# KennyRotella/delta_graph_slam

Measured on AMD Instinct MI355X. Metric: scan registrations/sec (64k-pt pairs), higher is better.
Workload: dtype f32 per-point, f64 accumulate; 1 GPU; cfg2 KITTI HDL-64E-shaped pairs (65,536 pts after voxel filter), NDT res 1.0 m DIRECT7, eps 0.01, max 64 iterations; 32 candidate pairs per GPU per step against one target (LoopDetector::matching, cfg4 shard), 32 distinct source scans, fitness score per candidate; inputs resident on the device before timing -- the 35 MB working set of a step fits the 256 MB Infinity Cache, so re-reads between eval; pairs_per_gpu=32, distinct_scans=32, parallelism=candidates sharded one process per GPU, all_gather of result records, collective_world_size=1

## Files before the change

delta_graph_slam_amd/csrc/dgs_api.hip:

```cpp
#include <algorithm>
#include <cfloat>
#include <cmath>
#include <cstddef>
#include <cstdlib>
#include <cstring>
#include <new>

#include "handle.h"

using namespace dgs;

namespace dgs {

int ensure_pinned(dgs_handle* h, size_t bytes) {
  if (bytes <= h->pinned_bytes) return DGS_OK;
  if (h->pinned) (void)hipHostFree(h->pinned);
  h->pinned = nullptr;
  h->pinned_bytes = 0;
  const size_t want = std::max<size_t>(bytes * 2, 1 << 16);
  hipError_t e = hipHostMalloc(&h->pinned, want, hipHostMallocDefault);
  if (e != hipSuccess) {
    h->err = std::string("hipHostMalloc: ") + hipGetErrorString(e);
    return DGS_ERR_HIP;
  }
// ... 252 lines not shown
  p->ndt_min_points_per_voxel = 6;
  p->ndt_line_search = DGS_NDT_LS_MORE_THUENTE;
  p->ndt_mt_max_step_iterations = 10;
  p->ndt_fix_hessian_d1 = 0;
  p->ndt_strict_order = DGS_NDT_ORDER_UPSTREAM;
  p->ndt_newton_solver = 1;
  p->ndt_hessian_recompute_double = 1;
  p->ndt_guess_rotation_polar = 1;
  p->ndt_exp_glibc = 1;
  p->ndt_cov_eigensolver = 1;
  p->gicp_cov_jacobi_svd = 0;
  p->gicp_max_correspondence_distance = 2.5;
  p->gicp_rotation_epsilon = 2e-3;
  p->gicp_lm_init_lambda_factor = 1e-9;
  p->gicp_correspondence_randomness = 20;
  p->gicp_regularization = DGS_GICP_REG_PLANE;
  p->gicp_optimizer = DGS_GICP_OPT_LEVENBERG_MARQUARDT;
  p->gicp_lm_max_iterations = 10;
  p->vgicp_search_method = DGS_VGICP_DIRECT1;
  p->vgicp_resolution = 1.0;
  if (method == DGS_METHOD_PCL_NDT) p->ndt_search_method = DGS_NDT_KDTREE;
  return valid_method(method) ? DGS_OK : DGS_ERR_INVALID_ARGUMENT;
}

int dgs_pcl_gicp_options_init(dgs_pcl_gicp_options* o) {
  if (!o) return DGS_ERR_INVALID_ARGUMENT;
  std::memset(o, 0, sizeof(*o));
  o->struct_size = sizeof(dgs_pcl_gicp_options);
  o->max_optimizer_iterations = 20;
  o->rotation_epsilon = 2e-3;
  o->gicp_epsilon = 1e-3;
  o->use_reciprocal_correspondences = 0;
  return DGS_OK;
}

int dgs_set_pcl_gicp_options(dgs_handle* h, const dgs_pcl_gicp_options* o) {
  if (!h || !o || o->struct_size != sizeof(dgs_pcl_gicp_options)) return DGS_ERR_INVALID_ARGUMENT;
  h->err.clear();
  if (h->prm.method != DGS_METHOD_PCL_GICP) { h->err = "dgs_set_pcl_gicp_options: not a GICP_HIP handle"; return DGS_ERR_UNSUPPORTED; }
  if (o->max_optimizer_iterations < 1 || !(o->rotation_epsilon > 0) || !(o->gicp_epsilon >= 0)) {
    h->err = "dgs_set_pcl_gicp_options: max_optimizer_iterations >= 1, rotation_epsilon > 0 and gicp_epsilon >= 0 are required";
    return DGS_ERR_INVALID_ARGUMENT;
  }
  h->pg_opt = *o;
  return DGS_OK;
}

int dgs_pcl_gicp_set_correspondence_randomness(dgs_handle* h, int32_t k) {
  if (!h || k < 1) return DGS_ERR_INVALID_ARGUMENT;
  h->err.clear();
  if (h->prm.method != DGS_METHOD_PCL_GICP) { h->err = "dgs_pcl_gicp_set_correspondence_randomness: not a GICP_HIP handle"; return DGS_ERR_UNSUPPORTED; }
  h->prm.gicp_correspondence_randomness = k;
  return DGS_OK;
}

int dgs_pcl_gicp_get_trajectory(dgs_handle* h, int32_t pair, float* T16s, int32_t* n_corr, int32_t* inner, int32_t* passes, double* f, int32_t capacity,
                                int32_t* len) {
  if (!h || !len || pair < 0 || capacity < 0) return DGS_ERR_INVALID_ARGUMENT;
  h->err.clear();
  if (set_device(h)) return DGS_ERR_HIP;
  if (h->prm.method != DGS_METHOD_PCL_GICP) return DGS_ERR_UNSUPPORTED;
  int n = 0;
  int rc = pcl_gicp_trajectory(h, pair, T16s, n_corr, inner, passes, f, capacity, &n);
  *len = n;
  return rc;
}

int dgs_pcl_gicp_set_probe(dgs_handle* h, const float* T16, const float* guess16) {
  if (!h) return DGS_ERR_INVALID_ARGUMENT;
  h->err.clear();
  if (h->prm.method != DGS_METHOD_PCL_GICP) return DGS_ERR_UNSUPPORTED;
  std::memcpy(h->pg_probe_T, T16 ? T16 : kIdentity16, sizeof(h->pg_probe_T));
  std::memcpy(h->pg_probe_guess, guess16 ? guess16 : kIdentity16, sizeof(h->pg_probe_guess));
  return DGS_OK;
}

int dgs_pcl_gicp_evaluate(dgs_handle* h, const double* x6, int32_t* m, double* f, double* g6) {
  if (!h || !x6 || !m || !f || !g6) return DGS_ERR_INVALID_ARGUMENT;
  h->err.clear();
  if (set_device(h)) return DGS_ERR_HIP;
  if (h->prm.method != DGS_METHOD_PCL_GICP) return DGS_ERR_UNSUPPORTED;
  if (!h->have_target || h->nt == 0) return DGS_ERR_NO_TARGET;
  if (!h->have_source || h->ns == 0) return DGS_ERR_NO_SOURCE;
  return pcl_gicp_evaluate(h, x6, m, f, g6);
}

int dgs_icp_options_init(dgs_icp_options* o) {
  if (!o) return DGS_ERR_INVALID_ARGUMENT;
  std::memset(o, 0, sizeof(*o));
  o->struct_size = sizeof(dgs_icp_options);
  o->use_reciprocal_correspondences = 0;
  o->euclidean_fitness_epsilon = -DBL_MAX;
  o->rotation_epsilon = 0.0;
  return DGS_OK;
}

int dgs_set_icp_options(dgs_handle* h, const dgs_icp_options* o) {
  if (!h || !o || o->struct_size != sizeof(dgs_icp_options)) return DGS_ERR_INVALID_ARGUMENT;
  h->err.clear();
  if (h->prm.method != DGS_METHOD_ICP) { h->err = "dgs_set_icp_options: not an ICP handle"; return DGS_ERR_UNSUPPORTED; }
  h->icp_opt = *o;
  return DGS_OK;
}

int dgs_icp_get_trajectory(dgs_handle* h, int32_t pair, float* T16s, double* mse, int32_t* n_corr, int32_t capacity, int32_t* len) {
  if (!h || !len || pair < 0 || capacity < 0) return DGS_ERR_INVALID_ARGUMENT;
  h->err.clear();
  if (set_device(h)) return DGS_ERR_HIP;
  if (h->prm.method != DGS_METHOD_ICP) return DGS_ERR_UNSUPPORTED;
  int n = 0;
  int rc = icp_trajectory(h, pair, T16s, mse, n_corr, capacity, &n);
  *len = n;
  return rc;
}

int dgs_create(const dgs_params* params, dgs_handle** out) {
  if (!params || !out || params->struct_size != sizeof(dgs_params)) return DGS_ERR_INVALID_ARGUMENT;
  if (!valid_method(params->method)) return DGS_ERR_INVALID_ARGUMENT;
  if (params->method == DGS_METHOD_VGICP && (!(params->vgicp_resolution > 0) || params->vgicp_search_method < 0 || params->vgicp_search_method > DGS_VGICP_DIRECT27))
    return DGS_ERR_INVALID_ARGUMENT;
  if (!(params->ndt_resolution > 0) || params->maximum_iterations < 0 || params->gicp_correspondence_randomness < 1) return DGS_ERR_INVALID_ARGUMENT;
  if (params->ndt_strict_order < DGS_NDT_ORDER_FAST || params->ndt_strict_order > DGS_NDT_ORDER_UPSTREAM_SEQUENTIAL) return DGS_ERR_INVALID_ARGUMENT;
  *out = nullptr;
  dgs_handle* h = new (std::nothrow) dgs_handle();
  if (!h) return DGS_ERR_HIP;
  h->prm = *params;
  if (params->method == DGS_METHOD_PCL_NDT) {
    h->prm.ndt_search_method = DGS_NDT_KDTREE;
    h->prm.ndt_strict_order = DGS_NDT_ORDER_UPSTREAM;
    h->prm.ndt_hessian_recompute_double = 1;
  }
  int dev = params->device;
  hipError_t e = hipSuccess;
  if (dev < 0) e = hipGetDevice(&dev);
  if (e == hipSuccess) e = hipSetDevice(dev);
  if (e == hipSuccess) e = hipStreamCreateWithFlags(&h->stream, hipStreamNonBlocking);
  if (e != hipSuccess) {
    g_create_error = std::string("dgs_create(device=") + std::to_string(params->device) + "): " + hipGetErrorString(e);
    delete h;
    return DGS_ERR_HIP;
  }
  h->device = dev;
  h->own_stream = true;
  (void)side_create(h);
  if (kExperiments)
    if (const char* e = std::getenv("DGS_NN_GRID")) { h->grid_mode = std::atoi(e); h->grid_levels = std::max(1, std::atoi(e)); }
  if (const char* e = std::getenv("DGS_NDT_FUSED")) h->ndt_fused = std::atoi(e) != 0;
  if (const char* e = std::getenv("DGS_NDT_STRICT_KERNEL")) h->strict_kernel = std::atoi(e) == 2 ? 2 : 3;
  if (const char* e = std::getenv("DGS_NDT_HD_OVERLAP")) h->hd_overlap = std::atoi(e) != 0;
  if (const char* e = std::getenv("DGS_NDT_SOLVE_MIN_ACTIVE")) h->solve_min_active = std::max(0, std::atoi(e));
  if (const char* e = std::getenv("DGS_NDT_SPECULATE")) h->ndt_speculate = std::atoi(e) != 0;
  if (const char* e = std::getenv("DGS_NDT_FIXED_SLICES")) h->ndt_fixed_slices = std::atoi(e) != 0;
  if (const char* e = std::getenv("DGS_NDT_DEAL_BY_COST")) h->ndt_deal_by_cost = std::atoi(e) != 0;
  if (const char* e = std::getenv("DGS_NDT_QUEUE")) h->ndt_queue_mode = std::atoi(e);
  if (const char* e = std::getenv("DGS_NDT_SCHEDULE")) h->ndt_schedule = std::atoi(e) != 0;
  if (const char* e = std::getenv("DGS_NDT_QUEUE_MIN_PAIRS")) h->ndt_queue_min_pairs = std::max(1, std::atoi(e));
  if (const char* e = std::getenv("DGS_EARLY_FITNESS")) h->early_fitness_enabled = std::atoi(e) != 0;
  if (const char* e = std::getenv("DGS_EARLY_FITNESS_LDS_KB")) h->early_fit.lds_kb = std::max(0, std::atoi(e));
  if (const char* e = std::getenv("DGS_EARLY_FITNESS_MAX_ACTIVE")) h->early_fit.max_active = std::max(0, std::atoi(e));
  if (const char* e = std::getenv("DGS_EARLY_FITNESS_MIN_PAIRS")) h->early_fit.min_pairs = std::max(1, std::atoi(e));
  if (const char* e = std::getenv("DGS_NN_KD")) h->nn_kd = std::atoi(e) != 0;
  if (const char* e = std::getenv("DGS_NN_KD_ALL")) h->nn_kd_all = std::atoi(e) != 0;
  if (const char* e = std::getenv("DGS_NN_KD_MIN_QUERIES")) h->nn_kd_min_queries = std::atoll(e);
  if (const char* e = std::getenv("DGS_KNN_PARTS")) { const int v = std::atoi(e); h->knn_parts = (v == 1 || v == 2 || v == 4 || v == 8) ? v : 0; }
  if (const char* e = std::getenv("DGS_KNN_LEAF")) h->knn_leaf = std::atoi(e) != 0;
  if (const char* e = std::getenv("DGS_KNN_MIN_WAVES")) h->knn_min_waves = std::max(1, std::atoi(e));
  if (const char* e = std::getenv("DGS_KNN_ROUNDS")) h->knn_rounds = std::max(1, std::atoi(e));
  if (const char* e = std::getenv("DGS_GICP_FUSED")) h->gicp_fused = std::atoi(e) != 0;
  if (kExperiments)
    if (const char* e = std::getenv("DGS_NDT_PACK2")) h->ndt_pack2 = std::atoi(e) != 0;
  if (const char* e = std::getenv("DGS_NN_GRID_FACTOR")) h->grid_spacing_factor = std::max(0.5f, (float)std::atof(e));
  std::memset(h->final_T, 0, sizeof(h->final_T));
  h->final_T[0] = h->final_T[5] = h->final_T[10] = h->final_T[15] = 1.f;
  (void)dgs_icp_options_init(&h->icp_opt);
  (void)dgs_pcl_gicp_options_init(&h->pg_opt);
  *out = h;
  return DGS_OK;
}

void dgs_destroy(dgs_handle* h) {
  if (!h) return;
  (void)hipSetDevice(h->device);
  (void)hipStreamSynchronize(h->stream);
  unbind(h, h->tgt_cloud);
  unbind(h, h->src_cloud);
  h->own_target.release(); h->own_source.release();
  for (int k = 0; k < 2; k++)
    if (h->ev_poll[k]) (void)hipEventDestroy(h->ev_poll[k]);
  if (h->hd_stream) {
    (void)hipStreamSynchronize(h->hd_stream);
    (void)hipStreamDestroy(h->hd_stream);
    for (int k = 0; k < dgs_handle::kHdEvents; k++) {
      if (h->ev_hd_a[k]) (void)hipEventDestroy(h->ev_hd_a[k]);
      if (h->ev_hd_b[k]) (void)hipEventDestroy(h->ev_hd_b[k]);
    }
  }
  if (h->side_stream) {
    (void)hipStreamSynchronize(h->side_stream);
    (void)hipStreamDestroy(h->side_stream);
    (void)hipEventDestroy(h->ev_fork);
    (void)hipEventDestroy(h->ev_join);
  }
  h->batch_slab.release();
  for (auto& c : h->batch_clouds) c.release();
  icp_release(h);
  pcl_gicp_release(h);
  prefilter_release(h);
  map_cloud_release(h);
  line_extraction_release(h);
  line_align_release(h);
  line_align_local_release(h);
  line_edges_release(h);
  building_overlap_release(h);
  floor_detection_release(h);
  fitness_batch_release(h);
  building_cloud_release(h);
  h->gitems.release(); h->vvox.release(); h->vcell2vox.release();
  h->cell2vox.release(); h->vox.release(); h->vox_centroid.release(); h->vox_dbg.release(); h->vox_strict.release(); h->vox_count.release(); h->vox_valid.release();
  h->key_in.release(); h->key_out.release(); h->val_in.release(); h->val_out.release(); h->run_keys.release();
  h->run_counts.release(); h->run_offsets.release(); h->dev_scalars.release(); h->vg_run_keys.release(); h->vg_scalars.release(); h->minmax_partial.release(); h->cub_temp.release();
  h->pairs.release(); h->inits.release(); h->partials.release(); h->done_counter.release(); h->ndt_queue.release(); h->ndt_ring.release(); h->pair_blocks.release(); h->src_ptrs.release(); h->src_sizes.release();
  h->nn_partials.release(); h->scratch_cloud.release(); h->strict_rows.release(); h->strict_totals.release(); h->tgt_grid.release(); h->aux_grid.release();
  h->fc_in.release(); h->fc_out.release(); h->fc_cnt.release();
  h->aux_cloud1.release(); h->aux_cloud2.release(); h->aux_out.release(); h->aux_bvh.release();
  h->corr.release(); h->corr_sq.release(); h->mahal.release(); h->gpairs.release(); h->slice_blk_pair.release(); h->slice_rows.release();
  for (auto& ep : h->prof.pool) { (void)hipEventDestroy(ep.start); (void)hipEventDestroy(ep.stop); }
  if (h->pinned) (void)hipHostFree(h->pinned);
  if (h->done_flags) (void)hipHostFree(h->done_flags);
  if (h->fit_host) (void)hipHostFree(h->fit_host);
  if (h->own_stream && h->stream) (void)hipStreamDestroy(h->stream);
  delete h;
}

const char* dgs_last_error(const dgs_handle* h) { return h ? h->err.c_str() : g_create_error.c_str(); }

int dgs_set_stream(dgs_handle* h, void* hip_stream) {
  if (!h) return DGS_ERR_INVALID_ARGUMENT;
  h->err.clear();
  if (set_device(h)) return DGS_ERR_HIP;
  DGS_HIP_TRY(h, hipStreamSynchronize(h->stream));
  if (h->own_stream && h->stream) (void)hipStreamDestroy(h->stream);
  if (hip_stream) {
    h->stream = reinterpret_cast<hipStream_t>(hip_stream);
    h->own_stream = false;
  } else {
    DGS_HIP_TRY(h, hipStreamCreateWithFlags(&h->stream, hipStreamNonBlocking));
    h->own_stream = true;
  }
  return DGS_OK;
}

int dgs_synchronize(dgs_handle* h) {
  if (!h) return DGS_ERR_INVALID_ARGUMENT;
  h->err.clear();
  if (set_device(h)) return DGS_ERR_HIP;
  DGS_HIP_TRY(h, hipStreamSynchronize(h->stream));
  return DGS_OK;
}

int dgs_set_input_target(dgs_handle* h, const float* xyz16, int64_t n, int32_t on_device) {
  if (!h || n < 0 || (n > 0 && !xyz16) || n > INT32_MAX) return DGS_ERR_INVALID_ARGUMENT;
  h->err.clear();
  if (set_device(h)) return DGS_ERR_HIP;
  h->have_target = false;
  h->vmap_valid = false;
  h->tgt_grid.valid = false;
  unbind(h, h->tgt_cloud);
  h->tgt = &h->own_target;
  h->tgt->invalidate();
  h->tgt->n = n;
  h->nt = n;
  int rc = upload_cloud(h, h->own_target.pts, xyz16, n, on_device);
  if (rc) return rc;
  if (is_ndt_family(h)) {
    rc = ndt_build_target(h);
    if (rc) return rc;
  }
  h->have_target = true;
  return DGS_OK;
}

int dgs_set_input_source(dgs_handle* h, const float* xyz16, int64_t n, int32_t on_device) {
  if (!h || n < 0 || (n > 0 && !xyz16) || n > INT32_MAX) return DGS_ERR_INVALID_ARGUMENT;
  h->err.clear();
  if (set_device(h)) return DGS_ERR_HIP;
  h->have_source = false;
  unbind(h, h->src_cloud);
  h->src = &h->own_source;
  h->src->invalidate();
  h->src->n = n;
  h->ns = n;
  int rc = upload_cloud(h, h->own_source.pts, xyz16, n, on_device);
  if (rc) return rc;
  h->have_source = true;
  return DGS_OK;
}

int dgs_cloud_create(dgs_handle* h, const float* xyz16, int64_t n, int32_t on_device, dgs_cloud** out) {
  if (!h || !out || n < 0 || (n > 0 && !xyz16) || n > INT32_MAX) return DGS_ERR_INVALID_ARGUMENT;
  h->err.clear();
  *out = nullptr;
  if (set_device(h)) return DGS_ERR_HIP;
  dgs_cloud* c = new (std::nothrow) dgs_cloud();
  if (!c) return DGS_ERR_HIP;
  c->device = h->device;
  c->st.n = n;
  int rc = upload_cloud(h, c->st.pts, xyz16, n, on_device);
  if (rc != DGS_OK) {
    c->st.release();
    delete c;
    return rc;
  }
  *out = c;
  return DGS_OK;
}

void dgs_cloud_destroy(dgs_cloud* c) {
  if (!c) return;
  for (dgs_handle* h : c->users) {
    if (h->tgt_cloud == c) { h->tgt_cloud = nullptr; h->tgt = &h->own_target; h->nt = 0; h->have_target = false; h->tgt_grid.valid = false; }
    if (h->src_cloud == c) { h->src_cloud = nullptr; h->src = &h->own_source; h->ns = 0; h->have_source = false; }
  }
  (void)hipSetDevice(c->device);
  (void)hipDeviceSynchronize();
  c->st.release();
  delete c;
}

int64_t dgs_cloud_size(const dgs_cloud* c) { return c ? c->st.n : 0; }

int dgs_set_input_target_cloud(dgs_handle* h, dgs_cloud* c) {
  if (!h || !c || c->device != h->device) return DGS_ERR_INVALID_ARGUMENT;
  h->err.clear();
  if (set_device(h)) return DGS_ERR_HIP;
  h->have_target = false;
  h->vmap_valid = false;
  h->tgt_grid.valid = false;
  bind(h, h->tgt_cloud, c);
  h->tgt = &c->st;
  h->nt = c->st.n;
  if (is_ndt_family(h)) {
    int rc = ndt_build_target(h);
    if (rc) return rc;
  }
  h->have_target = true;
  return DGS_OK;
}

int dgs_set_input_source_cloud(dgs_handle* h, dgs_cloud* c) {
  if (!h || !c || c->device != h->device) return DGS_ERR_INVALID_ARGUMENT;
  h->err.clear();
  bind(h, h->src_cloud, c);
  h->src = &c->st;
  h->ns = c->st.n;
  h->have_source = true;
  return DGS_OK;
}

static void fail_result(dgs_result* r, const float* guess, int status) {
  std::memcpy(r->final_transformation, guess ? guess : kIdentity16, sizeof(float) * 16);
  r->converged = 0;
  r->iterations = 0;
  r->evaluations = 0;
  r->status = status;
  r->score = 0.0;
  r->fitness = NAN;
}

int dgs_align(dgs_handle* h, const float* guess16, dgs_result* out, float* aligned, int32_t aligned_on_device) {
  if (!h || !out) return DGS_ERR_INVALID_ARGUMENT;
  h->err.clear();
  fail_result(out, guess16, DGS_OK);
  if (set_device(h)) { out->status = DGS_ERR_HIP; return DGS_ERR_HIP; }
// ... 49 lines not shown
  if (!h->have_target || h->nt == 0) return DGS_ERR_NO_TARGET;
  if (!h->have_source || h->ns == 0) return DGS_ERR_NO_SOURCE;
  double sum = 0;
  int64_t cnt = 0, inl = 0;
  int rc = nn_fitness(h, h->src->pts.ptr, h->ns, h->final_T, DBL_MAX, max_sq_dist, &sum, &cnt, &inl);
  if (rc) return rc;
  *fraction = (double)inl / (double)h->ns;
  return DGS_OK;
}

int dgs_nearest_search_target(dgs_handle* h, const float* queries, int64_t m, int32_t on_device, int32_t* indices, float* sq_dists) {
  if (!h || m < 0 || (m > 0 && (!queries || !indices || !sq_dists))) return DGS_ERR_INVALID_ARGUMENT;
  h->err.clear();
  if (set_device(h)) return DGS_ERR_HIP;
  if (!h->have_target || h->nt == 0) return DGS_ERR_NO_TARGET;
  if (m == 0) return DGS_OK;
  const float4* dq = reinterpret_cast<const float4*>(queries);
  int32_t* didx = indices;
  float* dsq = sq_dists;
  DevBuf<float4> q;
  DevBuf<int32_t> bi;
  DevBuf<float> bd;
  int rc = DGS_OK;
  if (!on_device) {
    if (q.reserve(m) != hipSuccess || bi.reserve(m) != hipSuccess || bd.reserve(m) != hipSuccess) { h->err = "hipMalloc failed"; rc = DGS_ERR_HIP; }
    if (!rc && hipMemcpyAsync(q.ptr, queries, (size_t)m * sizeof(float4), hipMemcpyHostToDevice, h->stream) != hipSuccess) { h->err = "hipMemcpyAsync failed"; rc = DGS_ERR_HIP; }
    dq = q.ptr; didx = bi.ptr; dsq = bd.ptr;
  }
  if (!rc) rc = nn_search(h, dq, m, didx, dsq);
  if (!rc && !on_device) {
    if (hipMemcpyAsync(indices, didx, (size_t)m * sizeof(int32_t), hipMemcpyDeviceToHost, h->stream) != hipSuccess ||
        hipMemcpyAsync(sq_dists, dsq, (size_t)m * sizeof(float), hipMemcpyDeviceToHost, h->stream) != hipSuccess) { h->err = "hipMemcpyAsync failed"; rc = DGS_ERR_HIP; }
  }
  (void)hipStreamSynchronize(h->stream);
  q.release(); bi.release(); bd.release();
  return rc;
}

int dgs_nn_fitness_distances(dgs_handle* h, const float* queries, int64_t m, int32_t on_device, float* sq_dists) {
  if (!h || m < 0 || (m > 0 && (!queries || !sq_dists))) return DGS_ERR_INVALID_ARGUMENT;
  h->err.clear();
  if (set_device(h)) return DGS_ERR_HIP;
  if (!h->have_target || h->nt == 0) return DGS_ERR_NO_TARGET;
  if (h->grid_mode == 0) return DGS_ERR_UNSUPPORTED;
  if (m == 0) return DGS_OK;
  h->use_grid = true;
  if (side_join(h) != DGS_OK) return DGS_ERR_HIP;
  int rc = ensure_target_index(h);
  if (rc) return rc;
  const float4* dq = reinterpret_cast<const float4*>(queries);
  float* dsq = sq_dists;
  DevBuf<float4> q;
  DevBuf<float> bd;
  if (!on_device) {
    if (q.reserve(m) != hipSuccess || bd.reserve(m) != hipSuccess) { h->err = "hipMalloc failed"; rc = DGS_ERR_HIP; }
    if (!rc && hipMemcpyAsync(q.ptr, queries, (size_t)m * sizeof(float4), hipMemcpyHostToDevice, h->stream) != hipSuccess) { h->err = "hipMemcpyAsync failed"; rc = DGS_ERR_HIP; }
    dq = q.ptr; dsq = bd.ptr;
  }
  if (!rc) rc = nn_grid_search(h, h->tgt_grid, h->tgt->bvh, dq, m, dsq);
  if (!rc && !on_device && hipMemcpyAsync(sq_dists, dsq, (size_t)m * sizeof(float), hipMemcpyDeviceToHost, h->stream) != hipSuccess) { h->err = "hipMemcpyAsync failed"; rc = DGS_ERR_HIP; }
  (void)hipStreamSynchronize(h->stream);
  q.release(); bd.release();
  return rc;
}

static int gicp_batch(dgs_handle* h, int n, CloudState* const* cs, const float* guesses16, int compute_fitness, double fitness_max_range,
                      dgs_result* results) {
  struct KdScope { dgs_handle* h; ~KdScope() { h->batch_kd = false; } } kd_scope{h};
  static const int kd_min = std::getenv("DGS_GICP_KD_MIN_CANDIDATES") ? std::atoi(std::getenv("DGS_GICP_KD_MIN_CANDIDATES")) : 10;
  h->batch_kd = h->nn_kd && n >= kd_min;
  const MethodOps& ops = kMethodOps[h->prm.method];
  int rc = ops.align_batch(h, n, cs, guesses16, results);
  if (rc == DGS_OK && compute_fitness) {
    DGS_HIP_TRY(h, h->src_ptrs.reserve(n));
    DGS_HIP_TRY(h, h->src_sizes.reserve(n));
    std::vector<const float4*> ptrs(n);
    std::vector<int> sz(n);
    int max_n = 0;
    for (int i = 0; i < n; i++) { ptrs[i] = cs[i]->pts.ptr; sz[i] = (int)cs[i]->n; max_n = std::max(max_n, sz[i]); }
    DGS_HIP_TRY(h, hipMemcpyAsync(h->src_ptrs.ptr, ptrs.data(), sizeof(void*) * n, hipMemcpyHostToDevice, h->stream));
    DGS_HIP_TRY(h, hipMemcpyAsync(h->src_sizes.ptr, sz.data(), sizeof(int) * n, hipMemcpyHostToDevice, h->stream));
    DGS_HIP_TRY(h, hipStreamSynchronize(h->stream));
    std::vector<double> sums(n);
    std::vector<int64_t> cnts(n), inl(n);
    size_t stride = 0;
    const float* dT = ops.final_transforms(h, &stride);
    rc = nn_fitness_batch(h, n, h->src_ptrs.ptr, h->src_sizes.ptr, max_n, dT, stride, fitness_max_range, 0.0, sums.data(), cnts.data(), inl.data());
    if (rc == DGS_OK)
      for (int i = 0; i < n; i++) results[i].fitness = cnts[i] > 0 ? sums[i] / (double)cnts[i] : DBL_MAX;
  }
  if (rc == DGS_OK) {
    for (int i = 0; i < n; i++)
      if (cs[i]->n <= 0) fail_result(&results[i], guesses16 ? guesses16 + 16 * i : nullptr, DGS_ERR_NO_SOURCE);
  }
  return rc;
}

int dgs_align_batch(dgs_handle* h, int32_t n, const float* const* sources, const int64_t* sizes, int32_t on_device, const float* guesses16,
                    int32_t compute_fitness, double fitness_max_range, dgs_result* results) {
  if (!h || n < 0 || (n > 0 && (!sources || !sizes || !results))) return DGS_ERR_INVALID_ARGUMENT;
  h->err.clear();
  if (set_device(h)) return DGS_ERR_HIP;
  if (n == 0) return DGS_OK;
  for (int i = 0; i < n; i++) fail_result(&results[i], guesses16 ? guesses16 + 16 * i : nullptr, DGS_OK);
  if (!h->have_target || h->nt == 0) {
    for (int i = 0; i < n; i++) results[i].status = DGS_ERR_NO_TARGET;
    h->err = "no input target dataset was given";
    return DGS_ERR_NO_TARGET;
  }
  if (!is_ndt_family(h)) {
    if (h->batch_clouds.size() < (size_t)n) h->batch_clouds.resize(n);
    std::vector<CloudState*> cs(n);
    for (int i = 0; i < n; i++) {
      if (sizes[i] < 0 || sizes[i] > INT32_MAX) return DGS_ERR_INVALID_ARGUMENT;
      CloudState& c = h->batch_clouds[i];
      c.invalidate();
      c.n = sources[i] ? sizes[i] : 0;
      int rc = upload_cloud(h, c.pts, sources[i], c.n, on_device);
      if (rc) return rc;
      cs[i] = &c;
    }
    return gicp_batch(h, n, cs.data(), guesses16, compute_fitness, fitness_max_range, results);
  }
  std::vector<const float4*> ptrs(n);
  std::vector<int> sz(n);
  DevBuf<float4>& slab = h->batch_slab;
  int64_t total = 0;
  for (int i = 0; i < n; i++) {
    if (sizes[i] < 0 || sizes[i] > INT32_MAX || (sizes[i] > 0 && !sources[i])) return DGS_ERR_INVALID_ARGUMENT;
    sz[i] = (int)sizes[i];
    total += sizes[i];
  }
  if (!on_device) {
    DGS_HIP_TRY(h, slab.reserve((size_t)std::max<int64_t>(total, 1)));
    int64_t off = 0;
    for (int i = 0; i < n; i++) {
      ptrs[i] = slab.ptr + off;
      if (sz[i]) DGS_HIP_TRY(h, hipMemcpyAsync(slab.ptr + off, sources[i], (size_t)sz[i] * sizeof(float4), hipMemcpyHostToDevice, h->stream));
      off += sz[i];
    }
  } else {
    for (int i = 0; i < n; i++) ptrs[i] = reinterpret_cast<const float4*>(sources[i]);
  }
  h->use_grid = grid_wanted(h, total);
  struct KdScope { dgs_handle* h; ~KdScope() { h->batch_kd = false; } } kd_scope{h};
  h->batch_kd = h->nn_kd && compute_fitness && total >= h->nn_kd_min_queries;
  if (compute_fitness && (!h->tgt->bvh.valid || (h->use_grid && !h->tgt_grid.valid)) && !h->prof.enabled) {
    int rs = side_fork(h);
    if (rs != DGS_OK) return rs;
    h->side_build_deferred = true;
  }
  int max_n = 0;
  for (int i = 0; i < n; i++) max_n = std::max(max_n, sz[i]);
  h->early_fit.on = h->early_fitness_enabled && compute_fitness && !h->prof.enabled && !h->use_grid && n <= 65535;
  h->early_fit.enqueued = false;
  h->early_fit.max_range = fitness_max_range;
  h->early_fit.max_n = max_n;
  int rc = ndt_align_pairs(h, n, ptrs.data(), sz.data(), guesses16, results);
  h->early_fit.on = false;
  if (side_join(h) != DGS_OK && rc == DGS_OK) rc = DGS_ERR_HIP;
  if (rc == DGS_OK && compute_fitness && h->early_fit.enqueued) {
    std::vector<double> sums(n);
    std::vector<int64_t> cnts(n), inl(n);
    nn_fitness_read(h, n, sums.data(), cnts.data(), inl.data());
    for (int i = 0; i < n; i++) results[i].fitness = cnts[i] > 0 ? sums[i] / (double)cnts[i] : DBL_MAX;
  } else if (rc == DGS_OK && compute_fitness) {
    std::vector<double> sums(n);
    std::vector<int64_t> cnts(n), inl(n);
    const float* dT = reinterpret_cast<const float*>(reinterpret_cast<const char*>(h->pairs.ptr) + offsetof(NdtPair, final_T));
    rc = nn_fitness_batch(h, n, h->src_ptrs.ptr, h->src_sizes.ptr, max_n, dT, sizeof(NdtPair), fitness_max_range, 0.0, sums.data(), cnts.data(),
                          inl.data());
    if (rc == DGS_OK)
      for (int i = 0; i < n; i++) results[i].fitness = cnts[i] > 0 ? sums[i] / (double)cnts[i] : DBL_MAX;
  }
  if (rc == DGS_OK) {
    for (int i = 0; i < n; i++)
      if (sz[i] == 0)
        fail_result(&results[i], guesses16 ? guesses16 + 16 * i : nullptr, DGS_ERR_NO_SOURCE);
  }
  (void)hipStreamSynchronize(h->stream);
  return rc;
}

int dgs_align_batch_clouds(dgs_handle* h, int32_t n, dgs_cloud* const* sources, const float* guesses16, int32_t compute_fitness,
                           double fitness_max_range, dgs_result* results) {
  if (!h || n < 0 || (n > 0 && (!sources || !results))) return DGS_ERR_INVALID_ARGUMENT;
  h->err.clear();
  if (set_device(h)) return DGS_ERR_HIP;
  if (n == 0) return DGS_OK;
  for (int i = 0; i < n; i++)
    if (!sources[i] || sources[i]->device != h->device) return DGS_ERR_INVALID_ARGUMENT;
  if (is_ndt_family(h)) {
    std::vector<const float*> ptrs(n);
    std::vector<int64_t> sizes(n);
    for (int i = 0; i < n; i++) { ptrs[i] = reinterpret_cast<const float*>(sources[i]->st.pts.ptr); sizes[i] = sources[i]->st.n; }
    return dgs_align_batch(h, n, ptrs.data(), sizes.data(), 1, guesses16, compute_fitness, fitness_max_range, results);
  }
  for (int i = 0; i < n; i++) fail_result(&results[i], guesses16 ? guesses16 + 16 * i : nullptr, DGS_OK);
  if (!h->have_target || h->nt == 0) {
    for (int i = 0; i < n; i++) results[i].status = DGS_ERR_NO_TARGET;
    h->err = "no input target dataset was given";
    return DGS_ERR_NO_TARGET;
  }
  std::vector<CloudState*> cs(n);
  for (int i = 0; i < n; i++) cs[i] = &sources[i]->st;
  return gicp_batch(h, n, cs.data(), guesses16, compute_fitness, fitness_max_range, results);
}

int dgs_profile_enable(dgs_handle* h, int32_t enable) {
  if (!h) return DGS_ERR_INVALID_ARGUMENT;
  if (set_device(h)) return DGS_ERR_HIP;
  prof_collect(h);
  h->prof.enabled = enable != 0;
  return DGS_OK;
}

int dgs_profile_get(dgs_handle* h, int32_t kernel_id, double* total_ms, int64_t* launches) {
  if (!h || kernel_id < 0 || kernel_id >= DGS_K_COUNT) return DGS_ERR_INVALID_ARGUMENT;
  if (set_device(h)) return DGS_ERR_HIP;
  prof_collect(h);
  if (total_ms) *total_ms = h->prof.total_ms[kernel_id];
  if (launches) *launches = h->prof.launches[kernel_id];
  return DGS_OK;
}

int dgs_profile_reset(dgs_handle* h) {
  if (!h) return DGS_ERR_INVALID_ARGUMENT;
  if (set_device(h)) return DGS_ERR_HIP;
  prof_collect(h);
  for (int k = 0; k < DGS_K_COUNT; k++) { h->prof.total_ms[k] = 0; h->prof.launches[k] = 0; }
  return DGS_OK;
}

int dgs_get_counts(dgs_handle* h, int64_t out[8]) {
  if (!h || !out) return DGS_ERR_INVALID_ARGUMENT;
  h->err.clear();
  if (set_device(h)) return DGS_ERR_HIP;
  for (int k = 0; k < 8; k++) out[k] = 0;
  out[0] = h->nt;
  out[1] = h->ns;
  if (is_ndt_family(h) && h->have_target && h->grid_cells > 0) {
    if (h->counts_stale) {
      int sc[2] = {0, 0};
      DGS_HIP_TRY(h, hipMemcpyAsync(sc, h->dev_scalars.ptr, sizeof(sc), hipMemcpyDeviceToHost, h->stream));
      DGS_HIP_TRY(h, hipStreamSynchronize(h->stream));
      h->n_occupied = sc[0];
      h->n_valid = sc[1];
      h->counts_stale = false;
    }
    out[2] = h->n_valid;
    out[3] = h->n_occupied;
    out[4] = h->grid_cells;
  }
  out[5] = h->last_evaluations;
  return DGS_OK;
}

int dgs_ndt_derivatives(dgs_handle* h, const double* p6, const float* T16, double* score, double* grad6, double* hess36) {
  if (!h || !p6 || !score || !grad6 || (!hess36 && !is_pcl_ndt(h))) return DGS_ERR_INVALID_ARGUMENT;
  h->err.clear();
  if (set_device(h)) return DGS_ERR_HIP;
  if (!is_ndt_family(h)) return DGS_ERR_UNSUPPORTED;
  if (!h->have_target || h->nt == 0) return DGS_ERR_NO_TARGET;
  if (!h->have_source || h->ns == 0) return DGS_ERR_NO_SOURCE;
  if (!hess36) {
    double unused[36];
    return ndt_probe(h, p6, T16, score, grad6, unused, 0);
  }
  return ndt_probe(h, p6, T16, score, grad6, hess36);
}

int dgs_pcl_ndt_neighbours(dgs_handle* h, const float* queries_xyz16, int64_t m, int32_t on_device, int32_t* counts, int32_t* voxel_ids) {
  if (!h || m < 0 || m > INT32_MAX || (m > 0 && (!queries_xyz16 || !counts || !voxel_ids))) return DGS_ERR_INVALID_ARGUMENT;
  h->err.clear();
  if (set_device(h)) return DGS_ERR_HIP;
  if (!is_pcl_ndt(h)) { h->err = "dgs_pcl_ndt_neighbours: not a PCL_NDT_HIP handle"; return DGS_ERR_UNSUPPORTED; }
  if (!h->have_target || h->nt == 0) return DGS_ERR_NO_TARGET;
  return pcl_ndt_neighbours(h, queries_xyz16, m, on_device, counts, voxel_ids);
}

int dgs_ndt_hessian_double(dgs_handle* h, const double* p6, double* hess36) {
  if (!h || !p6 || !hess36) return DGS_ERR_INVALID_ARGUMENT;
  h->err.clear();
  if (set_device(h)) return DGS_ERR_HIP;
  if (!is_ndt_family(h) || h->prm.ndt_strict_order == DGS_NDT_ORDER_FAST || !h->prm.ndt_hessian_recompute_double) return DGS_ERR_UNSUPPORTED;
  if (!h->have_target || h->nt == 0) return DGS_ERR_NO_TARGET;
  if (!h->have_source || h->ns == 0) return DGS_ERR_NO_SOURCE;
  double score, g6[6];
  return ndt_probe(h, p6, nullptr, &score, g6, hess36, 2);
}

int dgs_ndt_score_gradient(dgs_handle* h, const double* p6, double* score, double* grad6) {
  if (!h || !p6 || !score || !grad6) return DGS_ERR_INVALID_ARGUMENT;
  h->err.clear();
  if (set_device(h)) return DGS_ERR_HIP;
  if (!is_ndt_family(h) || is_pcl_ndt(h) || h->prm.ndt_strict_order == DGS_NDT_ORDER_FAST) return DGS_ERR_UNSUPPORTED;
  if (!h->have_target || h->nt == 0) return DGS_ERR_NO_TARGET;
  if (!h->have_source || h->ns == 0) return DGS_ERR_NO_SOURCE;
  double unused[36];
  return ndt_probe(h, p6, nullptr, score, grad6, unused, 0);
}

int dgs_deal_probe(dgs_handle* h, const int32_t* active, int32_t n_pairs, int32_t cap_blocks, int32_t grid, int32_t* out) {
  if (!h || !active || !out || n_pairs < 1 || cap_blocks < 1 || grid < n_pairs || grid > (1 << 20)) return DGS_ERR_INVALID_ARGUMENT;
  h->err.clear();
  if (set_device(h)) return DGS_ERR_HIP;
  DevBuf<int> d_active;
  DevBuf<int4> d_out;
  const size_t n_out = (size_t)grid * (kBlock / kWave);
  hipError_t e = d_active.reserve((size_t)n_pairs);
  if (e == hipSuccess) e = d_out.reserve(n_out);
  if (e == hipSuccess) e = hipMemcpyAsync(d_active.ptr, active, sizeof(int) * (size_t)n_pairs, hipMemcpyHostToDevice, h->stream);
  if (e == hipSuccess) {
    hipLaunchKernelGGL(deal_probe_kernel, dim3(grid), dim3(kBlock), 0, h->stream, d_active.ptr, n_pairs, cap_blocks, d_out.ptr);
    e = hipGetLastError();
  }
  if (e == hipSuccess) e = hipMemcpyAsync(out, d_out.ptr, sizeof(int4) * n_out, hipMemcpyDeviceToHost, h->stream);
  if (e == hipSuccess) e = hipStreamSynchronize(h->stream);
  d_active.release();
  d_out.release();
  if (e != hipSuccess) {
    h->err = std::string("dgs_deal_probe: ") + hipGetErrorString(e);
    return DGS_ERR_HIP;
  }
  return DGS_OK;
}

int dgs_deal_probe_cost(dgs_handle* h, const int32_t* active, const int32_t* kinds, int32_t n_pairs, int32_t cap_blocks, int32_t grid, int32_t* out, int32_t* order3) {
  if (!h || !active || !kinds || !out || n_pairs < 1 || cap_blocks < 1 || grid < n_pairs || grid > (1 << 20)) return DGS_ERR_INVALID_ARGUMENT;
  for (int32_t i = 0; i < n_pairs; i++)
    if (kinds[i] < 0 || kinds[i] > 2) return DGS_ERR_INVALID_ARGUMENT;
  h->err.clear();
  if (set_device(h)) return DGS_ERR_HIP;
  if (order3) { order3[0] = kNdtCostKind0; order3[1] = kNdtCostKind1; order3[2] = kNdtCostKind2; }
  DevBuf<int> d_in;
  DevBuf<int4> d_out;
  const size_t n_out = (size_t)grid * (kBlock / kWave);
  hipError_t e = d_in.reserve(2 * (size_t)n_pairs);
  if (e == hipSuccess) e = d_out.reserve(n_out);
  if (e == hipSuccess) e = hipMemcpyAsync(d_in.ptr, active, sizeof(int) * (size_t)n_pairs, hipMemcpyHostToDevice, h->stream);
  if (e == hipSuccess) e = hipMemcpyAsync(d_in.ptr + n_pairs, kinds, sizeof(int) * (size_t)n_pairs, hipMemcpyHostToDevice, h->stream);
  if (e == hipSuccess) {
    hipLaunchKernelGGL(deal_probe_cost_kernel, dim3(grid), dim3(kBlock), 0, h->stream, d_in.ptr, d_in.ptr + n_pairs, n_pairs, cap_blocks, d_out.ptr);
    e = hipGetLastError();
  }
  if (e == hipSuccess) e = hipMemcpyAsync(out, d_out.ptr, sizeof(int4) * n_out, hipMemcpyDeviceToHost, h->stream);
  if (e == hipSuccess) e = hipStreamSynchronize(h->stream);
  d_in.release();
  d_out.release();
  if (e != hipSuccess) {
    h->err = std::string("dgs_deal_probe_cost: ") + hipGetErrorString(e);
    return DGS_ERR_HIP;
  }
  return DGS_OK;
}

int dgs_find_loop_candidates(dgs_handle* h, const double* accum_distance, const double* xy, int64_t n, int32_t on_device, double new_accum_distance,
                             const double* new_xy, double accum_distance_thresh, double distance_thresh, int32_t* indices, int64_t capacity, int64_t* n_out) {
  if (!h || !n_out || !new_xy || n < 0 || capacity < 0 || (n > 0 && (!accum_distance || !xy)) || (capacity > 0 && !indices) || n > INT32_MAX) return DGS_ERR_INVALID_ARGUMENT;
  h->err.clear();
  if (set_device(h)) return DGS_ERR_HIP;
  *n_out = 0;
  if (n == 0) return DGS_OK;
  dgs::DevBuf<double>& din = h->fc_in;
  dgs::DevBuf<int>& dout = h->fc_out;
  dgs::DevBuf<long long>& dcnt = h->fc_cnt;
  const double* d_acc = accum_distance;
  const double* d_xy = xy;
  int* d_idx = indices;
  const int64_t cap = on_device ? capacity : std::min<int64_t>(capacity, n);
  if (dcnt.reserve(1) != hipSuccess) { h->err = "hipMalloc failed"; return DGS_ERR_HIP; }
  if (ensure_pinned(h, 8192) != DGS_OK) return DGS_ERR_HIP;
  long long* count = reinterpret_cast<long long*>(reinterpret_cast<char*>(h->pinned) + 4096);
  *count = 0;
  if (!on_device) {
    if (din.reserve((size_t)3 * n) != hipSuccess || dout.reserve((size_t)std::max<int64_t>(cap, 1)) != hipSuccess) { h->err = "hipMalloc failed"; return DGS_ERR_HIP; }
    DGS_HIP_TRY(h, hipMemcpyAsync(din.ptr, accum_distance, sizeof(double) * n, hipMemcpyHostToDevice, h->stream));
    DGS_HIP_TRY(h, hipMemcpyAsync(din.ptr + n, xy, sizeof(double) * 2 * n, hipMemcpyHostToDevice, h->stream));
    d_acc = din.ptr; d_xy = din.ptr + n; d_idx = dout.ptr;
  }
  hipLaunchKernelGGL(find_candidates_kernel, dim3(1), dim3(1024), 0, h->stream, d_acc, d_xy, (long long)n, new_accum_distance, new_xy[0], new_xy[1],
                     accum_distance_thresh, distance_thresh, d_idx, (long long)cap, dcnt.ptr);
  DGS_HIP_TRY(h, hipMemcpyAsync(count, dcnt.ptr, sizeof(long long), hipMemcpyDeviceToHost, h->stream));
  if (!on_device && cap > 0) DGS_HIP_TRY(h, hipMemcpyAsync(indices, d_idx, sizeof(int32_t) * (size_t)cap, hipMemcpyDeviceToHost, h->stream));
  DGS_HIP_TRY(h, hipStreamSynchronize(h->stream));
  if (hipGetLastError() != hipSuccess) { h->err = "find_candidates_kernel failed"; return DGS_ERR_HIP; }
  *n_out = *count;
  if (*count > capacity) { h->err = "indices buffer too small for the candidates"; return DGS_ERR_INVALID_ARGUMENT; }
  return DGS_OK;
}

int dgs_calc_fitness_score(dgs_handle* h, const float* cloud1, int64_t n1, const float* cloud2, int64_t n2, int32_t on_device,
                           const float* relpose16, double max_range, double* score) {
  if (!h || !score || n1 < 0 || n2 < 0 || (n1 > 0 && !cloud1) || (n2 > 0 && !cloud2) || n1 > INT32_MAX || n2 > INT32_MAX) return DGS_ERR_INVALID_ARGUMENT;
  h->err.clear();
  if (set_device(h)) return DGS_ERR_HIP;
  *score = DBL_MAX;
  if (n1 == 0 || n2 == 0) return DGS_OK;
  int rc = upload_cloud(h, h->aux_cloud1, cloud1, n1, on_device);
  if (rc == DGS_OK) rc = upload_cloud(h, h->aux_cloud2, cloud2, n2, on_device);
  if (rc == DGS_OK) rc = bvh_build(h, h->aux_bvh, h->aux_cloud1.ptr, n1);
  const bool aux_grid = grid_wanted(h, n2);
  if (rc == DGS_OK && aux_grid) rc = nn_grid_build(h, h->aux_grid, h->aux_bvh, h->aux_cloud1.ptr, n1);
  if (rc != DGS_OK) return rc;
  hipStream_t st = h->stream;
// ... 172 lines not shown
```

delta_graph_slam_amd/csrc/handle.h:

```cpp
#pragma once
#include "building_cloud.h"
#include "common.h"
#include "sac.h"

namespace dgs {

struct EventPair {
  hipEvent_t start, stop;
};

struct Profiler {
  bool enabled = false;
  std::vector<EventPair> pool;
  std::vector<int> pending[DGS_K_COUNT];
  size_t next_free = 0;
  double total_ms[DGS_K_COUNT] = {0};
  int64_t launches[DGS_K_COUNT] = {0};
};

struct IcpPair;
struct IcpItem;
struct PgPair;
struct PgItem;
struct PgInit;
// ... 134 lines not shown
  DevBuf<LaHyp> hyps;
  DevBuf<unsigned char> keep, gate;
  DevBuf<int> blk, cnt, surv, slot;
  DevBuf<double> fit;
  DevBuf<LaResult> result;
  int64_t n_hyp = 0;
  int64_t counts4[4] = {0, 0, 0, 0};
};
struct LalHyp;
struct LalScratch {
  DevBuf<unsigned char> in;
  DevBuf<unsigned char> tab;
  DevBuf<LalHyp> hyps;
  DevBuf<double> fit;
  DevBuf<double> keys;
  DevBuf<double> base;
  DevBuf<unsigned char> out;
  std::vector<int64_t> off1, off2;
  int64_t counts8[8] = {0, 0, 0, 0, 0, 0, 0, 0};
};
struct LeSeg;
struct LeScratch {
  DevBuf<double> lines;
  DevBuf<LeSeg> segs;
  DevBuf<unsigned char> cnt;
  DevBuf<int> blk;
  DevBuf<int> eoff;
  DevBuf<double> edges;
  void* stage = nullptr;
  size_t stage_bytes = 0;
  std::vector<int> eoff_host;
  int64_t counts4[4] = {0, 0, 0, 0};
};
struct BoHyp;
struct BoScratch {
  DevBuf<unsigned char> in;
  DevBuf<double> shr;
  DevBuf<unsigned long long> bits;
  DevBuf<int> row;
  DevBuf<unsigned char> out;
  DevBuf<unsigned char> ain;
  DevBuf<BoHyp> hyps;
  DevBuf<unsigned char> aout;
  std::vector<int64_t> off;
  int64_t counts8[8] = {0, 0, 0, 0, 0, 0, 0, 0};
};

struct FdHyp;
struct FdScratch {
  DevBuf<float4> in, tilted, clipped, kept, filtered;
  DevBuf<unsigned char> flags, nflags;
  DevBuf<int> blk, cnt;
  CloudState cloud;
  DevBuf<int> nbr;
  DevBuf<float4> normals;
  DevBuf<float> cov9;
  SacScratch sac;
  DevBuf<FdHyp> hyps;
  std::vector<float4> host_filtered;
  std::vector<int32_t> inliers;
  int64_t n_clipped = 0, n_filtered = 0;
  bool have_normals = false;
  dgs_floor_detection_trace trace{};
};

struct FbEdge;
struct FbSeg;
struct FbScratch {
  DevBuf<unsigned char> tab;
  DevBuf<double> rows;
  void* stage = nullptr;
  size_t stage_bytes = 0;
  DevBuf<FbSeg> segs;
  DevBuf<float> mm;
  DevBuf<unsigned long long> keys, keys_alt;
  DevBuf<uint32_t> vals, vals_alt;
  void* bstage = nullptr;
  size_t bstage_bytes = 0;
  hipEvent_t ev_bstage = nullptr;
  bool bstage_pending = false;
  int64_t counts8[8] = {0, 0, 0, 0, 0, 0, 0, 0};
};

struct BcScratch {
  bc::StepTable steps;
  int64_t table_on_device = 0;
  DevBuf<float> table;
  DevBuf<unsigned char> in;
  DevBuf<float4> rec;
  DevBuf<int> cnt;
  DevBuf<int> item_off;
  DevBuf<float4> out;
  int64_t n_out = 0, n_items = -1;
  int64_t counts8[8] = {0, 0, 0, 0, 0, 0, 0, 0};
};

}

struct dgs_handle;
struct dgs_cloud {
  dgs::CloudState st;
  int device = 0;
  std::vector<dgs_handle*> users;
};

struct dgs_handle {
  dgs_params prm;
  int device = 0;
  hipStream_t stream = nullptr;
  bool own_stream = false;
  hipEvent_t ev_poll[2] = {nullptr, nullptr};
  hipStream_t side_stream = nullptr;
  hipEvent_t ev_fork = nullptr, ev_join = nullptr;
  hipStream_t hd_stream = nullptr;
  static constexpr int kHdEvents = 32;
  hipEvent_t ev_hd_a[kHdEvents] = {}, ev_hd_b[kHdEvents] = {};
  int strict_kernel = 3;
  bool hd_overlap = true;
  bool ndt_speculate = true;
  bool ndt_fixed_slices = false;
  bool ndt_deal_by_cost = true;
#ifdef DGS_DEAL_STAMPS
  unsigned long long* deal_stamps = nullptr;
  long long deal_stamp_seq = 0;
#endif
  int solve_min_active = 0;
  bool side_pending = false;
  bool side_build_deferred = false;
  std::string err;

  dgs::CloudState own_target, own_source;
  dgs::CloudState* tgt = &own_target;
  dgs::CloudState* src = &own_source;
  dgs_cloud* tgt_cloud = nullptr;
  dgs_cloud* src_cloud = nullptr;
  int64_t nt = 0, ns = 0;
  bool have_target = false, have_source = false;

  dgs::VoxelGrid grid{};
  dgs::DevBuf<int> cell2vox;
  dgs::DevBuf<dgs::VoxelRec> vox;
  dgs::DevBuf<float4> vox_centroid;
  dgs::DevBuf<double> vox_dbg;
  dgs::DevBuf<dgs::VoxelStrictRec> vox_strict;
  dgs::DevBuf<int> vox_count;
  dgs::DevBuf<int> vox_valid;
  dgs::DevBuf<uint32_t> key_in, key_out, val_in, val_out, run_keys;
  dgs::DevBuf<int> run_counts, run_offsets;
  dgs::DevBuf<int> dev_scalars;
  dgs::DevBuf<uint32_t> vg_run_keys;
  dgs::DevBuf<int> vg_scalars;
  dgs::DevBuf<float> minmax_partial;
  dgs::DevBuf<unsigned char> cub_temp;
  int64_t grid_cells = 0;
  int64_t n_occupied = 0, n_valid = 0;
  int64_t n_occupied_bound = 0;
  bool counts_stale = true;

  dgs::DevBuf<dgs::NdtPair> pairs;
  dgs::DevBuf<dgs::NdtInit> inits;
  dgs::DevBuf<double> partials;
  dgs::DevBuf<int> done_counter;
  int* done_flags = nullptr;
  int done_flags_cap = 0;
  dgs::DevBuf<int> ndt_queue;
  dgs::DevBuf<unsigned char> ndt_ring;
  int ndt_ring_rounds = 0;
  int ndt_queue_mode = 0;
  bool ndt_schedule = false;
  int ndt_queue_min_pairs = 2;
  dgs::DevBuf<int> pair_blocks;
  dgs::DevBuf<double> strict_rows;
  dgs::DevBuf<double> strict_totals;
  dgs::DevBuf<const float4*> src_ptrs;
  dgs::DevBuf<int> src_sizes;
  dgs::NdtConsts consts{};
  int64_t last_evaluations = 0;
  dgs::DevBuf<int> knn_nbr;
  dgs::DevBuf<int> knn_stats;
  bool nn_kd = true;
  int64_t nn_kd_min_queries = 6 * 65536;
  bool nn_kd_all = false;
  bool batch_kd = false;
  int knn_parts = 0;
  bool knn_leaf = true;
  int knn_min_waves = 4096;
  int knn_rounds = 8;
  bool gicp_fused = true;
  bool ndt_pack2 = false;
  bool ndt_fused = true;

  void* pinned = nullptr;
  size_t pinned_bytes = 0;

  float final_T[16];
  bool have_result = false;

  dgs::DevBuf<double> nn_partials;
  int nn_bpp = 0;
  double* fit_host = nullptr;
  int fit_host_cap = 0;
  struct EarlyFitness {
    bool on = false;
    bool enqueued = false;
    double max_range = 0.0;
    int max_n = 0;
    int lds_kb = 0;
    int max_active = 1 << 30;
    int min_pairs = 8;
  } early_fit;
  bool early_fitness_enabled = false;
  const double* nn_out = nullptr;
  dgs::DevBuf<float4> scratch_cloud;
  dgs::NnGrid tgt_grid, aux_grid;
  int grid_mode = 0;
  bool use_grid = false;
  int grid_levels = 1;
  float grid_spacing_factor = 6.f;

  dgs::DevBuf<float4> aux_cloud1, aux_cloud2, aux_out;
  dgs::DevBuf<double> fc_in;
  dgs::DevBuf<int> fc_out;
  dgs::DevBuf<long long> fc_cnt;
  dgs::Bvh aux_bvh;
  int64_t bvh_builds = 0;

  dgs::DevBuf<int> corr;
  dgs::DevBuf<float> corr_sq;
  dgs::DevBuf<double> mahal;
  dgs::DevBuf<dgs::GicpPair> gpairs;
  dgs::DevBuf<dgs::GicpItem> gitems;
  dgs::VgicpMap vmap{};
  dgs::DevBuf<dgs::VgicpVoxel> vvox;
  dgs::DevBuf<int> vcell2vox;
  bool vmap_valid = false;
  int64_t vmap_voxels = 0;
  dgs::DevBuf<float4> batch_slab;
  std::vector<dgs::CloudState> batch_clouds;
  dgs::GicpConsts gconsts{};

  dgs::DevBuf<int> slice_blk_pair;
  dgs::DevBuf<double> slice_rows;

  dgs_icp_options icp_opt{};
  dgs::DevBuf<dgs::IcpPair> ipairs;
  dgs::DevBuf<dgs::IcpItem> iitems;
  dgs::DevBuf<float4> icp_w;
  dgs::DevBuf<int> icp_origin;
  dgs::DevBuf<float> icp_traj_T;
  dgs::DevBuf<double> icp_traj_mse;
  dgs::DevBuf<int> icp_traj_n;
  std::vector<dgs::Bvh> icp_w_bvh;
  std::vector<int> icp_last_iters;
  int icp_traj_cap = 0;

  dgs_pcl_gicp_options pg_opt{};
  dgs::DevBuf<dgs::PgPair> pgpairs;
  dgs::DevBuf<dgs::PgItem> pgitems;
  dgs::DevBuf<dgs::PgInit> pginits;
  dgs::DevBuf<float4> pg_w;
  dgs::DevBuf<float4> pg_q;
  dgs::DevBuf<double> pg_m;
  dgs::DevBuf<float> pg_traj_T;
  dgs::DevBuf<int> pg_traj_i;
  dgs::DevBuf<double> pg_traj_f;
  std::vector<int> pg_last_iters;
  int pg_traj_cap = 0;
  float pg_probe_T[16] = {1, 0, 0, 0, 0, 1, 0, 0, 0, 0, 1, 0, 0, 0, 0, 1};
  float pg_probe_guess[16] = {1, 0, 0, 0, 0, 1, 0, 0, 0, 0, 1, 0, 0, 0, 0, 1};

  dgs::PfScratch pf;

  dgs::McScratch mc;

  dgs::LnScratch ln;
  dgs::LaScratch la;
  dgs::LalScratch lal;
  dgs::LeScratch le;
  dgs::BoScratch bo;

  dgs::FdScratch fd;

  dgs::FbScratch fb;

  dgs::BcScratch bcl;

  dgs::Profiler prof;
};

namespace dgs {

int prof_begin(dgs_handle* h, int kernel_id, hipStream_t st = nullptr);
void prof_end(dgs_handle* h, int kernel_id, int slot, hipStream_t st = nullptr);
int ensure_pinned(dgs_handle* h, size_t bytes);
int ensure_poll_events(dgs_handle* h);
int side_fork(dgs_handle* h);
int side_join(dgs_handle* h);
int side_build_now(dgs_handle* h);

int ndt_build_target(dgs_handle* h);
int voxel_grid_filter(dgs_handle* h, const float4* in, int64_t n, float leaf, float4* out, int64_t out_capacity, int64_t* n_out);
int approx_voxel_grid_filter(dgs_handle* h, const float4* in, int64_t n, float leaf, float4* out, int64_t out_capacity, int64_t* n_out);
int cloud_minmax(dgs_handle* h, const float4* pts, int64_t n, float out6[6]);
int cloud_minmax_device(dgs_handle* h, const float4* pts, int64_t n, float** d_out6, hipStream_t st = nullptr);
int ndt_align_pairs(dgs_handle* h, int n_pairs, const float4* const* d_src_ptrs_host, const int* sizes_host,
                    const float* guesses16, dgs_result* results);
int ndt_trajectory(dgs_handle* h, int pair, double* out, int* len);
int ndt_probe(dgs_handle* h, const double* p6, const float* T16, double* score, double* g6, double* H36, int kind = 1);
inline bool is_pcl_ndt(const dgs_handle* h) { return h->prm.method == DGS_METHOD_PCL_NDT; }
inline bool is_ndt_family(const dgs_handle* h) { return h->prm.method == DGS_METHOD_NDT || h->prm.method == DGS_METHOD_PCL_NDT; }
void pcl_ndt_launch(dgs_handle* h, int n_pairs, int cap_blocks, int total_blocks, int launch, hipStream_t st);
void pcl_ndt_init_tables(dgs_handle* h, int n_pairs, hipStream_t st);
int pcl_ndt_neighbours(dgs_handle* h, const float* queries_xyz16, int64_t m, int on_device, int32_t* counts, int32_t* voxel_ids);
int bvh_build(dgs_handle* h, Bvh& bvh, const float4* pts, int64_t n, hipStream_t st = nullptr, bool kd_order = false);
int nn_fitness(dgs_handle* h, const float4* src, int64_t n, const float* T16, double max_range, double inlier_sq,
               double* sum, int64_t* count, int64_t* inliers);
int nn_fitness_batch(dgs_handle* h, int n_pairs, const float4* const* d_src_ptrs, const int* d_sizes, int max_size, const float* d_T,
                     size_t T_stride_bytes, double max_range, double inlier_sq, double* sums, int64_t* counts, int64_t* inliers);
int nn_fitness_batch_on(dgs_handle* h, const Bvh& index, NnGrid* grid, int n_pairs, const float4* const* d_src_ptrs, const int* d_sizes, int max_size,
                        const float* d_T, size_t T_stride_bytes, double max_range, double inlier_sq, double* sums, int64_t* counts, int64_t* inliers);
int nn_fitness_prepare(dgs_handle* h, int n_pairs, int max_size, bool grid);
void nn_fitness_enqueue(dgs_handle* h, hipStream_t st, const Bvh& index, const int* ids, int count, const float4* const* d_src_ptrs, const int* d_sizes,
                        const float* d_T, size_t T_stride_bytes, double max_range, double inlier_sq, int background_lds_kb);
int nn_fitness_totals_enqueue(dgs_handle* h, int n_pairs);
void nn_fitness_read(const dgs_handle* h, int n_pairs, double* sums, int64_t* counts, int64_t* inliers);
int nn_search(dgs_handle* h, const float4* queries, int64_t m, int32_t* d_idx, float* d_sq);
int ensure_target_index(dgs_handle* h, hipStream_t st = nullptr);
inline bool grid_wanted(const dgs_handle* h, int64_t queries) { return h->grid_mode > 0 || (h->grid_mode < 0 && queries >= 262144); }
#ifdef DGS_EXPERIMENTS
constexpr bool kExperiments = true;
int nn_grid_build(dgs_handle* h, NnGrid& G, const Bvh& bvh, const float4* pts, int64_t n, hipStream_t st = nullptr);
int nn_grid_launch_fitness(dgs_handle* h, NnGrid& G, const Bvh& index, int n_pairs, const float4* const* d_src_ptrs, const int* d_sizes, int max_n, const float* d_T,
                           size_t T_stride_bytes, float max_range, float inlier_sq, double* partial, int bpp);
int nn_grid_search(dgs_handle* h, NnGrid& G, const Bvh& index, const float4* queries, int64_t m, float* d_sq);
#else
constexpr bool kExperiments = false;
inline int nn_grid_build(dgs_handle*, NnGrid&, const Bvh&, const float4*, int64_t, hipStream_t = nullptr) { return DGS_ERR_UNSUPPORTED; }
inline int nn_grid_launch_fitness(dgs_handle*, NnGrid&, const Bvh&, int, const float4* const*, const int*, int, const float*, size_t, float, float, double*, int) { return DGS_ERR_UNSUPPORTED; }
inline int nn_grid_search(dgs_handle*, NnGrid&, const Bvh&, const float4*, int64_t, float*) { return DGS_ERR_UNSUPPORTED; }
#endif
int vgicp_build_map(dgs_handle* h);
int vgicp_voxels(dgs_handle* h, int64_t capacity, int32_t* coord3, int32_t* counts, double* mean3, double* cov9, int64_t* n_voxels);
int gicp_ensure_target_covariance(dgs_handle* h);
int gicp_align(dgs_handle* h, const float* guess16, dgs_result* out);
int gicp_align_batch(dgs_handle* h, int n, CloudState* const* srcs, const float* guesses16, dgs_result* out);
const float* gicp_final_transforms(dgs_handle* h, size_t* stride_bytes);
int gicp_covariances(dgs_handle* h, int which, double* host_out6, int64_t n);
int gicp_probe(dgs_handle* h, const double* T16_rowmajor, int error_only, double* err, double* H36, double* b6);
int icp_align(dgs_handle* h, const float* guess16, dgs_result* out);
int icp_align_batch(dgs_handle* h, int n, CloudState* const* srcs, const float* guesses16, dgs_result* out);
const float* icp_final_transforms(dgs_handle* h, size_t* stride_bytes);
int icp_trajectory(dgs_handle* h, int pair, float* T16s, double* mse, int32_t* n_corr, int capacity, int* len);
void icp_release(dgs_handle* h);
int knn_lists(dgs_handle* h, CloudState& c, int k, DevBuf<int>* out = nullptr);
void prefilter_release(dgs_handle* h);
void map_cloud_release(dgs_handle* h);
// ... 25 lines not shown
```

delta_graph_slam_amd/csrc/ndt_align.hip:

```cpp
#include <cfloat>
#include <cmath>
#include <cstdlib>
#include <cstring>

#include "handle.h"
#include "ndt_plan.h"
#include "solve6.h"

namespace dgs {

#include "ndt_fast.h"

#pragma clang fp contract(off)

#include "ndt_exp_tables.h"
#include "ndt_optimiser.h"
#include "ndt_strict.h"
#include "ndt_sequential.h"

__host__ __device__ inline int ndt_queue_slices(int round, int base, int cap) {
  const int f = round < 12 ? 1 : (round < 24 ? 2 : 4);
  return min(base * f, cap);
}
constexpr int kQueueHdrWords = 82;
static_assert(offsetof(NdtPair, need_hessian) == 81 * 4, "header layout");
constexpr size_t kQueueSlotBytes = 384;
__host__ __device__ inline NdtPair* queue_slot(char* ring, int ring_rounds, int pair, int round) {
  return reinterpret_cast<NdtPair*>(ring + ((size_t)pair * ring_rounds + round) * kQueueSlotBytes);
}
__device__ __forceinline__ unsigned long long* queue_word(int* queue, int pair) { return reinterpret_cast<unsigned long long*>(queue) + 1 + pair; }
__device__ __forceinline__ unsigned long long* queue_ctl(int* queue) { return reinterpret_cast<unsigned long long*>(queue); }
constexpr int kQueueStatInts = 16;

__global__ void ndt_init_kernel(NdtPair* __restrict__ pairs, const NdtInit* __restrict__ inits, int n_pairs, const NdtConsts c, int probe,
                                int* __restrict__ done_counter, const float4* const* __restrict__ stage_ptrs, const int* __restrict__ stage_sizes,
                                const float4** __restrict__ src_ptrs, int* __restrict__ src_sizes, int* __restrict__ queue, const int queue_slices0,
                                char* __restrict__ ring, const int ring_rounds) {
  const int i = blockIdx.x * blockDim.x + threadIdx.x;
  if (i < 16) done_counter[i] = 0;
  if (queue && i == 0) *queue_ctl(queue) = (unsigned long long)n_pairs;
  if (queue && i < kQueueStatInts) queue[2 * (n_pairs + 2) + i] = 0;
  if (i >= n_pairs) return;
  if (queue) *queue_word(queue, i) = (unsigned long long)queue_slices0 << 32;
  src_ptrs[i] = stage_ptrs[i];
  src_sizes[i] = stage_sizes[i];
  NdtPair* st = pairs + i;
  const NdtInit& in = inits[i];
  NdtSolver s;
  s.phase = probe ? PH_PROBE : PH_INIT_EVAL;
  s.nr_iterations = 0;
  s.trial_n = 0;
  s.trial_next = 0;
  s.evaluations = 0;
  s.converged = 0;
  s.step_iterations = 0;
  s.interval_converged = 0;
  s.open_interval = 1;
  s.traj_len = 1;
  s.score = 0;
  s.phi_0 = s.d_phi_0 = s.a_t = s.a_l = s.f_l = s.g_l = s.a_u = s.f_u = s.g_u = s.step_init = 0;
  for (int k = 0; k < 6; k++) { s.p[k] = in.p0[k]; s.grad[k] = 0; s.dir[k] = 0; st->traj[0][k] = in.p0[k]; }
  for (int k = 0; k < 36; k++) s.hess[k] = 0;
  double x[6];
  for (int k = 0; k < 6; k++) x[k] = in.p0[k];
  write_evaluation<false>(st, st, s, c, x, probe == 2 ? 2 : (probe == 3 ? 0 : 1), false, true);
  const float* G = in.guess;
  st->T[0] = G[0]; st->T[1] = G[4]; st->T[2] = G[8];  st->T[3] = G[12];
  st->T[4] = G[1]; st->T[5] = G[5]; st->T[6] = G[9];  st->T[7] = G[13];
  st->T[8] = G[2]; st->T[9] = G[6]; st->T[10] = G[10]; st->T[11] = G[14];
  for (int k = 0; k < 16; k++) st->final_T[k] = G[k];
  st->s = s;
  st->active = 1;
  st->last_launch = 0x7FFFFFFF;
  st->ticket = 0;
  st->serve[0] = 0;
  st->serve[1] = -1;
  st->serve[2] = -1;
  st->serve[3] = st->need_hessian & 3;
  st->spec_pending = 0;
  st->spec_result = 0;
  if (queue) {
    const int* from = reinterpret_cast<const int*>(st);
    int* to = reinterpret_cast<int*>(queue_slot(ring, ring_rounds, i, 0));
    for (int k = 0; k < kQueueHdrWords; k++) to[k] = from[k];
  }
}

struct NdtOut {
  float T[16];
  int converged, iterations, evaluations, pad;
  double score;
};

__global__ void ndt_export_kernel(const NdtPair* __restrict__ pairs, int n_pairs, NdtOut* __restrict__ out) {
  const int i = blockIdx.x * blockDim.x + threadIdx.x;
  if (i >= n_pairs) return;
  const NdtPair& st = pairs[i];
  NdtOut o;
  for (int k = 0; k < 16; k++) o.T[k] = st.final_T[k];
  o.converged = (st.s.phase == PH_DONE) ? st.s.converged : 0;
  o.iterations = st.s.nr_iterations;
  o.evaluations = st.s.evaluations;
  o.pad = 0;
  o.score = st.s.score;
  out[i] = o;
}

static void euler_angles_012(const float* T, float res[3]) {
  auto m = [&](int r, int c) { return T[c * 4 + r]; };
  const float kPi = 3.14159265358979323846f;
  res[0] = std::atan2(m(1, 2), m(2, 2));
  const float c2 = std::sqrt(m(0, 0) * m(0, 0) + m(0, 1) * m(0, 1));
  if (res[0] > 0.0f) {
    res[0] -= kPi;
    res[1] = std::atan2(-m(0, 2), -c2);
  } else {
    res[1] = std::atan2(-m(0, 2), c2);
  }
  const float s1 = std::sin(res[0]), c1 = std::cos(res[0]);
  res[2] = std::atan2(s1 * m(2, 0) - c1 * m(1, 0), c1 * m(1, 1) - s1 * m(2, 1));
  res[0] = -res[0];
  res[1] = -res[1];
  res[2] = -res[2];
}

static void affine_rotation_f32(const float* T_colmajor16, float* R) {
  constexpr int N = 3;
  const float precision = 2.f * FLT_EPSILON, tiny = FLT_MIN;
  float W[9], U[9], V[9];
  float scale = 0.f;
  for (int r = 0; r < 3; r++)
    for (int c = 0; c < 3; c++) { W[r * 3 + c] = T_colmajor16[c * 4 + r]; scale = std::fabs(W[r * 3 + c]) > scale ? std::fabs(W[r * 3 + c]) : scale; }
  if (scale == 0.f) scale = 1.f;
  for (int i = 0; i < 9; i++) { W[i] = W[i] / scale; U[i] = V[i] = (i % 4 == 0) ? 1.f : 0.f; }
  float max_diag = 0.f;
  for (int i = 0; i < N; i++) { const float a = std::fabs(W[i * 4]); if (a > max_diag) max_diag = a; }
  bool finished = false;
  for (int sweep = 0; sweep < 64 && !finished; sweep++) {
    finished = true;
    for (int p = 1; p < N; p++)
      for (int q = 0; q < p; q++) {
        const float pm = precision * max_diag;
        const float threshold = tiny > pm ? tiny : pm;
        if (!(std::fabs(W[p * N + q]) > threshold || std::fabs(W[q * N + p]) > threshold)) continue;
        finished = false;
        float m00 = W[p * N + p], m01 = W[p * N + q], m10 = W[q * N + p], m11 = W[q * N + q];
        const float t = m00 + m11, d = m10 - m01;
        float r1c, r1s;
        if (std::fabs(d) < tiny) { r1s = 0.f; r1c = 1.f; }
        else {
          const float u = t / d;
          const float tmp = std::sqrt(1.f + u * u);
          r1s = 1.f / tmp;
          r1c = u / tmp;
        }
        if (!(r1c == 1.f && r1s == 0.f)) {
          const float x0 = m00, y0 = m10, x1 = m01, y1 = m11;
          m00 = r1c * x0 + r1s * y0; m10 = -r1s * x0 + r1c * y0;
          m01 = r1c * x1 + r1s * y1; m11 = -r1s * x1 + r1c * y1;
        }
        float jrc, jrs;
        {
          const float deno = 2.f * std::fabs(m01);
          if (deno < tiny) { jrc = 1.f; jrs = 0.f; }
          else {
            const float tau = (m00 - m11) / deno;
            const float w = std::sqrt(tau * tau + 1.f);
            const float tt = (tau > 0.f) ? 1.f / (tau + w) : 1.f / (tau - w);
            const float sign_t = tt > 0.f ? 1.f : -1.f;
            const float nn = 1.f / std::sqrt(tt * tt + 1.f);
            jrs = -sign_t * (m01 / std::fabs(m01)) * std::fabs(tt) * nn;
            jrc = nn;
          }
        }
        const float jtc = jrc, jts = -jrs;
        const float jlc = r1c * jtc - r1s * jts;
        const float jls = r1c * jts + r1s * jtc;
        if (!(jlc == 1.f && jls == 0.f)) {
          for (int i = 0; i < N; i++) {
            const float xi = W[p * N + i], yi = W[q * N + i];
            W[p * N + i] = jlc * xi + jls * yi;
            W[q * N + i] = -jls * xi + jlc * yi;
          }
          for (int i = 0; i < N; i++) {
            const float xi = U[i * N + p], yi = U[i * N + q];
            U[i * N + p] = jlc * xi + jls * yi;
            U[i * N + q] = -jls * xi + jlc * yi;
          }
        }
        if (!(jrc == 1.f && -jrs == 0.f)) {
          const float c = jrc, s = -jrs;
// ... 125 lines not shown

#ifdef DGS_DEAL_STAMPS
static int deal_stamp_slot(dgs_handle* h, hipStream_t st) {
  static const char* file = std::getenv("DGS_DEAL_STAMPS_FILE");
  static const long long at = std::getenv("DGS_DEAL_STAMPS_AT") ? std::atoll(std::getenv("DGS_DEAL_STAMPS_AT")) : 2200;
  if (!file) return 0;
  const size_t words = (size_t)kStampLaunches * kStampGrid * kStampWords;
  const long long seq = h->deal_stamp_seq++;
  if (seq == at) {
    if (hipMalloc(reinterpret_cast<void**>(&h->deal_stamps), words * 8) != hipSuccess) { h->deal_stamps = nullptr; return 0; }
    (void)hipMemsetAsync(h->deal_stamps, 0, words * 8, st);
    (void)hipMemcpyToSymbolAsync(HIP_SYMBOL(g_deal_stamps), &h->deal_stamps, sizeof(h->deal_stamps), 0, hipMemcpyHostToDevice, st);
    (void)hipStreamSynchronize(st);
  }
  if (!h->deal_stamps || seq < at) return 0;
  if (seq < at + kStampLaunches) return (int)(seq - at) + 1;
  if (seq == at + kStampLaunches) {
    (void)hipStreamSynchronize(st);
    std::vector<unsigned long long> host(words);
    if (hipMemcpy(host.data(), h->deal_stamps, words * 8, hipMemcpyDeviceToHost) == hipSuccess) {
      if (FILE* f = std::fopen(file, "wb")) {
        std::fwrite(host.data(), 8, words, f);
        std::fclose(f);
      }
    }
  }
  return 0;
}
#endif

template <int SEARCH, bool FUSED, bool FIXED>
static void launch_strict_items(dgs_handle* h, const NdtPlan& P, const NdtLaunch& L, const dim3 grid, const int leaf_pow2, const int launch, hipStream_t st) {
  const int spec = (FUSED && P.speculate) ? 1 : 0;
  const dim3 grid_s(grid.x + (spec ? L.n_pairs : 0));
  int flags = (spec ? kStrictSpeculate : 0) | (h->ndt_deal_by_cost ? kStrictDealByCost : 0);
#ifdef DGS_DEAL_STAMPS
  flags |= deal_stamp_slot(h, st) << kStrictStampShift;
#endif
  hipLaunchKernelGGL((ndt_strict3_kernel<SEARCH, FUSED, true, FIXED>), grid_s, dim3(kBlock), 0, st, h->src_ptrs.ptr, h->src_sizes.ptr, h->pairs.ptr, h->grid, h->vox_strict.ptr,
                     h->vox_dbg.ptr, h->consts.gauss_d1, h->consts.gauss_d2, leaf_pow2, h->partials.ptr, L.n_pairs, L.cap_blocks, h->pair_blocks.ptr, h->consts,
                     FUSED ? h->done_flags : h->done_counter.ptr, launch, (FUSED && P.solve_beside) ? h->solve_min_active : 0, flags);
}

template <int SEARCH, bool FUSED, bool HD>
static void launch_strict_lanes(dgs_handle* h, const NdtPlan& P, const NdtLaunch& L, const dim3 grid, const int leaf_pow2, const int launch, hipStream_t st) {
  const int hd_lag = (FUSED && P.hd_overlap) ? 2 : 1;
  hipLaunchKernelGGL((ndt_strict_kernel<SEARCH, FUSED, HD>), grid, dim3(kBlock), 0, st, h->src_ptrs.ptr, h->src_sizes.ptr, h->pairs.ptr, h->grid, h->vox_strict.ptr,
                     h->vox_dbg.ptr, h->consts.gauss_d1, h->consts.gauss_d2, leaf_pow2, h->partials.ptr, L.n_pairs, L.cap_blocks, h->pair_blocks.ptr, h->consts,
                     FUSED ? h->done_flags : h->done_counter.ptr, launch, hd_lag);
}

template <int SEARCH, bool FUSED, bool PACK>
static void launch_fast(dgs_handle* h, const NdtLaunch& L, const dim3 grid, const int leaf_pow2, const int launch, hipStream_t st) {
  hipLaunchKernelGGL((ndt_derivatives_kernel<SEARCH, FUSED, PACK>), grid, dim3(kBlock), 0, st, h->src_ptrs.ptr, h->src_sizes.ptr, h->pairs.ptr, h->grid, h->consts.gauss_d1,
                     (float)h->consts.gauss_d2, leaf_pow2, h->partials.ptr, L.n_pairs, L.cap_blocks, h->pair_blocks.ptr, h->consts,
                     FUSED ? h->done_flags : h->done_counter.ptr, launch);
}

static void launch_derivatives(dgs_handle* h, const NdtPlan& P, const NdtLaunch& L, int launch = -1, bool hd = false) {
  const dim3 grid(L.total_blocks);
  int fe = 0;
  const int leaf_pow2 = (std::frexp(h->grid.leaf, &fe) == 0.5f) ? 1 : 0;
  const hipStream_t st = launch_stream(h, P, launch, hd);
  int slot = prof_begin(h, DGS_K_NDT_DERIVATIVES, st);
  if (is_pcl_ndt(h)) {
    if (!(hd && launch >= 0)) pcl_ndt_launch(h, L.n_pairs, L.cap_blocks, L.total_blocks, launch, st);
    prof_end(h, DGS_K_NDT_DERIVATIVES, slot, st);
    return;
  }
  with_search(P.search, [&](auto S) {
    constexpr int SEARCH = decltype(S)::value;
    if (P.order == DGS_NDT_ORDER_UPSTREAM_SEQUENTIAL) {
      launch_strict_rows<SEARCH>(h, L, grid, leaf_pow2, st);
    } else if (P.order == DGS_NDT_ORDER_UPSTREAM && P.item_kernel) {
      if (hd && launch >= 0) return;
      with_bool(launch >= 0, [&](auto FUSED) {
        with_bool(P.fixed_slices, [&](auto FIXED) { launch_strict_items<SEARCH, decltype(FUSED)::value, decltype(FIXED)::value>(h, P, L, grid, leaf_pow2, launch, st); });
      });
    } else if (P.order == DGS_NDT_ORDER_UPSTREAM) {
      with_bool(launch >= 0, [&](auto FUSED) {
        with_bool(hd, [&](auto HD) { launch_strict_lanes<SEARCH, decltype(FUSED)::value, decltype(HD)::value>(h, P, L, grid, leaf_pow2, launch, st); });
      });
    } else {
      with_bool(launch >= 0, [&](auto FUSED) {
        if constexpr (kExperiments && SEARCH == DGS_NDT_DIRECT7) {
          if (h->ndt_pack2) {
            launch_fast<SEARCH, decltype(FUSED)::value, true>(h, L, grid, leaf_pow2, launch, st);
            return;
          }
        }
        launch_fast<SEARCH, decltype(FUSED)::value, false>(h, L, grid, leaf_pow2, launch, st);
      });
    }
  });
  prof_end(h, DGS_K_NDT_DERIVATIVES, slot, st);
}

static void launch_solve(dgs_handle* h, const NdtPlan& P, const NdtLaunch& L) {
  int slot = prof_begin(h, DGS_K_NDT_SOLVE);
  hipLaunchKernelGGL(ndt_solve_kernel, dim3(L.n_pairs), dim3(kBlock), 0, h->stream, h->pairs.ptr, h->partials.ptr, L.cap_blocks, h->pair_blocks.ptr, h->consts,
                     h->done_counter.ptr, P.order != DGS_NDT_ORDER_FAST ? h->strict_totals.ptr : nullptr, P.order == DGS_NDT_ORDER_UPSTREAM ? 1 : 0);
  prof_end(h, DGS_K_NDT_SOLVE, slot);
}

static NdtLaunch choose_launch(int n_pairs, int max_n) {
  NdtLaunch L;
  L.n_pairs = n_pairs;
  static const int env_cap = std::getenv("DGS_NDT_CAP") ? std::atoi(std::getenv("DGS_NDT_CAP")) : 1024;
  static const int env_total = std::getenv("DGS_NDT_BLOCKS") ? std::atoi(std::getenv("DGS_NDT_BLOCKS")) : 1024;
  static const int env_ppt = std::getenv("DGS_NDT_PPT") ? std::max(1, std::atoi(std::getenv("DGS_NDT_PPT"))) : 2;
  static const int env_min = std::getenv("DGS_NDT_MIN_BLOCKS") ? std::max(1, std::atoi(std::getenv("DGS_NDT_MIN_BLOCKS"))) : 64;
  const int by_points = (max_n + kBlock * env_ppt - 1) / (kBlock * env_ppt);
  const int at_least = std::min(env_min, (max_n + kBlock - 1) / kBlock);
  L.cap_blocks = std::max(1, std::min({std::max(by_points, at_least), env_cap, kMaxPartialBlocks}));
  L.total_blocks = (int)std::max<int64_t>(n_pairs, std::min<int64_t>((int64_t)n_pairs * L.cap_blocks, env_total));
  L.max_n = std::max(max_n, 1);
  L.queue_workers = 0;
  L.queue_base = 0;
  return L;
}

static void choose_queue(dgs_handle* h, NdtLaunch& L) {
  static const int env_workers = std::getenv("DGS_NDT_QUEUE_WORKERS") ? std::atoi(std::getenv("DGS_NDT_QUEUE_WORKERS")) : 768;
  static const int env_base = std::getenv("DGS_NDT_QUEUE_BASE") ? std::atoi(std::getenv("DGS_NDT_QUEUE_BASE")) : 0;
  const int64_t most = (int64_t)L.n_pairs * L.cap_blocks;
  L.queue_workers = (int)std::max<int64_t>(1, std::min<int64_t>(env_workers, most));
  L.queue_base = env_base > 0 ? std::min(env_base, L.cap_blocks) : std::max(1, std::min(L.cap_blocks, L.queue_workers / std::max(1, L.n_pairs)));
  (void)h;
}

static int ndt_setup(dgs_handle* h, int n_pairs, const float4* const* src_ptrs_host, const int* sizes_host, const float* guesses16,
                     const double* probe_p6, NdtLaunch* launch_out, bool use_queue = false, int probe_kind = 1) {
  hipStream_t st = h->stream;
  fill_consts(h);
  int max_n = 0;
  for (int i = 0; i < n_pairs; i++) max_n = std::max(max_n, sizes_host[i]);
  NdtLaunch L = choose_launch(n_pairs, max_n);
  if (use_queue) {
    choose_queue(h, L);
    DGS_HIP_TRY(h, h->ndt_queue.reserve(2 * ((size_t)n_pairs + 2) + kQueueStatInts));
    const int per_iter_q = (h->prm.ndt_line_search == DGS_NDT_LS_FIXED_STEP && h->prm.ndt_step_size - h->prm.transformation_epsilon / 2 > 0) ? 1 : (h->prm.ndt_mt_max_step_iterations + 2);
    h->ndt_ring_rounds = (h->prm.maximum_iterations + 3) * per_iter_q + 8;
    DGS_HIP_TRY(h, h->ndt_ring.reserve((size_t)n_pairs * h->ndt_ring_rounds * kQueueSlotBytes));
  }
  *launch_out = L;
  DGS_HIP_TRY(h, h->pairs.reserve(n_pairs));
  DGS_HIP_TRY(h, h->inits.reserve(n_pairs));
  DGS_HIP_TRY(h, h->src_ptrs.reserve(n_pairs));
  DGS_HIP_TRY(h, h->src_sizes.reserve(n_pairs));
  DGS_HIP_TRY(h, h->partials.reserve((size_t)n_pairs * L.cap_blocks * (h->consts.strict_order ? kStrictPad : kAccumPad)));
  if (h->consts.strict_order) DGS_HIP_TRY(h, h->strict_totals.reserve((size_t)n_pairs * kStrictPad));
  if (h->consts.strict_order == DGS_NDT_ORDER_UPSTREAM_SEQUENTIAL) DGS_HIP_TRY(h, h->strict_rows.reserve((size_t)n_pairs * strict_rows_pair_stride(h, L)));
  DGS_HIP_TRY(h, h->pair_blocks.reserve(n_pairs));
  if (h->consts.strict_order == DGS_NDT_ORDER_UPSTREAM) DGS_HIP_TRY(h, hipMemsetAsync(h->pair_blocks.ptr, 0, sizeof(int) * n_pairs, st));
  DGS_HIP_TRY(h, h->done_counter.reserve(16));
  const size_t off_init = 256;
  const size_t off_ptr = off_init + sizeof(NdtInit) * n_pairs;
  const size_t off_size = off_ptr + sizeof(void*) * n_pairs;
  const size_t off_out = (off_size + sizeof(int) * n_pairs + 255) & ~(size_t)255;
  const size_t total = off_out + sizeof(NdtOut) * n_pairs + sizeof(NdtPair) + 256;
  if (ensure_pinned(h, total) != DGS_OK) return DGS_ERR_HIP;
  char* base = reinterpret_cast<char*>(h->pinned);
  NdtInit* hin = reinterpret_cast<NdtInit*>(base + off_init);
  const float ident[16] = {1, 0, 0, 0, 0, 1, 0, 0, 0, 0, 1, 0, 0, 0, 0, 1};
  for (int i = 0; i < n_pairs; i++) {
    const float* G = guesses16 ? guesses16 + 16 * i : ident;
    std::memcpy(hin[i].guess, G, sizeof(float) * 16);
    if (probe_p6) {
      for (int k = 0; k < 6; k++) hin[i].p0[k] = probe_p6[k];
    } else {
      float e[3];
      if (h->prm.ndt_guess_rotation_polar) {
        float R[9], Gp[16];
        affine_rotation_f32(G, R);
        std::memcpy(Gp, G, sizeof(Gp));
        for (int r = 0; r < 3; r++)
          for (int c = 0; c < 3; c++) Gp[c * 4 + r] = R[r * 3 + c];
        euler_angles_012(Gp, e);
      } else {
        euler_angles_012(G, e);
      }
      hin[i].p0[0] = G[12]; hin[i].p0[1] = G[13]; hin[i].p0[2] = G[14];
      hin[i].p0[3] = e[0]; hin[i].p0[4] = e[1]; hin[i].p0[5] = e[2];
    }
  }
  std::memcpy(base + off_ptr, src_ptrs_host, sizeof(void*) * n_pairs);
  std::memcpy(base + off_size, sizes_host, sizeof(int) * n_pairs);
  const size_t stage_bytes = off_size + sizeof(int) * n_pairs - off_init;
  DGS_HIP_TRY(h, h->inits.reserve((stage_bytes + sizeof(NdtInit) - 1) / sizeof(NdtInit)));
  DGS_HIP_TRY(h, hipMemcpyAsync(h->inits.ptr, hin, stage_bytes, hipMemcpyHostToDevice, st));
  const char* dstage = reinterpret_cast<const char*>(h->inits.ptr);
  hipLaunchKernelGGL(ndt_init_kernel, dim3((n_pairs + 63) / 64), dim3(64), 0, st, h->pairs.ptr, h->inits.ptr, n_pairs, h->consts, probe_p6 ? probe_kind : 0,
                     h->done_counter.ptr, reinterpret_cast<const float4* const*>(dstage + (off_ptr - off_init)),
                     reinterpret_cast<const int*>(dstage + (off_size - off_init)), h->src_ptrs.ptr, h->src_sizes.ptr,
                     L.queue_workers > 0 ? h->ndt_queue.ptr : nullptr, L.queue_workers > 0 ? ndt_queue_slices(0, L.queue_base, L.cap_blocks) : 0,
                     reinterpret_cast<char*>(h->ndt_ring.ptr), h->ndt_ring_rounds);
  if (is_pcl_ndt(h)) pcl_ndt_init_tables(h, n_pairs, st);
  return DGS_OK;
}

#ifdef DGS_EXPERIMENTS
#include "ndt_queue.h"
#else
static void launch_queue(dgs_handle*, const NdtLaunch&) {}
#endif

static int ndt_export(dgs_handle* h, int n_pairs, dgs_result* results);

int ndt_align_pairs(dgs_handle* h, int n_pairs, const float4* const* src_ptrs_host, const int* sizes_host, const float* guesses16,
                    dgs_result* results) {
  hipStream_t st = h->stream;
  NdtLaunch L{};
  const bool use_queue = kExperiments && h->ndt_queue_mode != 0 && h->ndt_fused && (h->consts.strict_order == DGS_NDT_ORDER_FAST) && n_pairs >= h->ndt_queue_min_pairs;
  int rc = ndt_setup(h, n_pairs, src_ptrs_host, sizes_host, guesses16, nullptr, &L, use_queue);
  if (rc != DGS_OK) return rc;
  const NdtPlan P = plan_align(h);
  if (use_queue) {
    launch_queue(h, L);
    if ((rc = side_build_now(h)) != DGS_OK) return rc;
    int* hq = reinterpret_cast<int*>(h->pinned);
    DGS_HIP_TRY(h, hipMemcpyAsync(hq, h->ndt_queue.ptr, sizeof(int) * 2, hipMemcpyDeviceToHost, st));
    rc = ndt_export(h, n_pairs, results);
    if (rc != DGS_OK) return rc;
#ifdef DGS_QUEUE_STATS
    {
      int q[8];
      (void)hipMemcpy(q, h->ndt_queue.ptr + 2 * (n_pairs + 2), sizeof(q), hipMemcpyDeviceToHost);
      int q2[8];
      (void)hipMemcpy(q2, h->ndt_queue.ptr + 2 * (n_pairs + 2) + 8, sizeof(q2), hipMemcpyDeviceToHost);
      const double it = std::max(1, q[4]);
      std::fprintf(stderr, "[queue] workers %d base %d: polls %d failed_claims %d claims %d closings %d; per worker: looking for work %.1f us, in items %.1f us; per item: %.2f us = record %.2f + "
                   "points %.2f + row %.2f + ticket %.2f; per closing %.2f us\n",
                   L.queue_workers, L.queue_base, q[2], q[3], q[4], q[7], q[5] * 0.01 / L.queue_workers, q[6] * 0.01 / L.queue_workers, q[6] * 0.01 / it, q2[0] * 0.01 / it,
                   q2[1] * 0.01 / it, q2[2] * 0.01 / it, q2[3] * 0.01 / it, q2[4] * 0.01 / std::max(1, q[7]));
    }
#endif
    if (hq[1] != 0 || hq[0] != 0) {
      h->err = "ndt_queue_kernel gave up (poll guard): " + std::to_string(hq[0]) + " registrations unfinished";
      return DGS_ERR_HIP;
    }
    return DGS_OK;
  }

  if (h->early_fit.on && (rc = nn_fitness_prepare(h, n_pairs, h->early_fit.max_n, false)) != DGS_OK) return rc;
  volatile int* flags = reinterpret_cast<volatile int*>(h->pinned);
  flags[0] = flags[1] = 0;
  if (ensure_poll_events(h) != DGS_OK) return DGS_ERR_HIP;
  const bool fused_flags = P.fused;
  if (fused_flags) {
    if (h->done_flags_cap < n_pairs) {
      if (h->done_flags) (void)hipHostFree(h->done_flags);
      h->done_flags = nullptr;
      h->done_flags_cap = 0;
      DGS_HIP_TRY(h, hipHostMalloc(reinterpret_cast<void**>(&h->done_flags), sizeof(int) * (size_t)(n_pairs + 64), hipHostMallocDefault));
      h->done_flags_cap = n_pairs + 64;
    }
    for (int i = 0; i < n_pairs; i++) h->done_flags[i] = 0;
  }
  hipEvent_t* ev = h->ev_poll;
  const bool fixed_one = h->prm.ndt_line_search == DGS_NDT_LS_FIXED_STEP && h->prm.ndt_step_size - h->prm.transformation_epsilon / 2 > 0;
  const int per_iter = fixed_one ? 1 : (h->prm.ndt_mt_max_step_iterations + 2);
  const long max_evals = ((long)(h->prm.maximum_iterations + 3) * per_iter + 2) * P.evals_factor;
  const int chunk = 4;
  long queued = 0;
  int launch_no = 0;
  const bool schedule = h->ndt_schedule;
  NdtLaunch Lq = L;
  if (schedule) choose_queue(h, Lq);
  int round_no = 0;
  int launches_upto[2] = {0, 0};
  int hd_rounds = 0;
  auto chained_round = [&](const NdtLaunch& Lr, auto&& beside) -> int {
    constexpr int R = dgs_handle::kHdEvents;
    if (launch_no >= 2) DGS_HIP_TRY(h, hipStreamWaitEvent(st, h->ev_hd_b[(launch_no - 2) % R], 0));
    launch_derivatives(h, P, Lr, launch_no);
    DGS_HIP_TRY(h, hipEventRecord(h->ev_hd_a[launch_no % R], st));
    DGS_HIP_TRY(h, hipStreamWaitEvent(h->hd_stream, h->ev_hd_a[launch_no % R], 0));
    beside();
    DGS_HIP_TRY(h, hipEventRecord(h->ev_hd_b[launch_no % R], h->hd_stream));
    hd_rounds = launch_no + 1;
    return DGS_OK;
  };
  auto enqueue_chunk = [&](int slot, int launches) -> int {
    for (int e = 0; e < launches; e++) {
      NdtLaunch Lr = L;
      if (schedule) {
        Lr.cap_blocks = ndt_queue_slices(round_no, Lq.queue_base, L.cap_blocks);
        Lr.total_blocks = n_pairs * Lr.cap_blocks;
      }
      round_no++;
      if (P.fused) {
        int rc_round = DGS_OK;
        if (P.two_kinds && P.hd_overlap) {
          rc_round = chained_round(Lr, [&] { launch_derivatives(h, P, Lr, launch_no, true); });
        } else if (P.solve_beside) {
          rc_round = chained_round(Lr, [&] {
            hipLaunchKernelGGL(ndt_strict_solve_kernel, dim3(n_pairs), dim3(kWave), 0, h->hd_stream, h->pairs.ptr, n_pairs, h->consts, h->done_flags, launch_no, 2);
          });
        } else {
          launch_derivatives(h, P, Lr, launch_no);
          if (P.two_kinds) launch_derivatives(h, P, Lr, launch_no, true);
        }
        if (rc_round != DGS_OK) return rc_round;
        launch_no++;
      } else {
        launch_derivatives(h, P, Lr);
        launch_solve(h, P, Lr);
        if (P.two_kinds) {
          launch_derivatives(h, P, Lr, -1, true);
          launch_solve(h, P, Lr);
        }
      }
    }
    queued += launches;
    launches_upto[slot] = launch_no;
    if (!fused_flags) DGS_HIP_TRY(h, hipMemcpyAsync(const_cast<int*>(&flags[slot]), h->done_counter.ptr, sizeof(int), hipMemcpyDeviceToHost, st));
    DGS_HIP_TRY(h, hipEventRecord(ev[slot], st));
    return DGS_OK;
  };
  auto pairs_done = [&](int slot) -> int {
    if (!fused_flags) return flags[slot];
    int n = 0;
    for (int i = 0; i < n_pairs; i++) n += reinterpret_cast<volatile int*>(h->done_flags)[i] != 0;
    return n;
  };
  const bool early = h->early_fit.on && fused_flags;
  std::vector<char> walked(early ? n_pairs : 0, 0);
  const float* fit_T = reinterpret_cast<const float*>(reinterpret_cast<const char*>(h->pairs.ptr) + offsetof(NdtPair, final_T));
  std::vector<int> ready;
  auto walk_finished = [&](int completed, bool rest) -> int {
    ready.clear();
    for (int i = 0; i < n_pairs; i++) {
      if (walked[i]) continue;
      const int f = reinterpret_cast<volatile int*>(h->done_flags)[i];
      if (rest || (f != 0 && f <= completed)) ready.push_back(i);
    }
    if (ready.empty() || (!rest && ((int)ready.size() < h->early_fit.min_pairs || n_pairs - pairs_done(0) > h->early_fit.max_active))) return DGS_OK;
    for (int i : ready) walked[i] = 1;
    nn_fitness_enqueue(h, rest ? st : h->side_stream, h->tgt->bvh, ready.data(), (int)ready.size(), h->src_ptrs.ptr, h->src_sizes.ptr, fit_T, sizeof(NdtPair),
                       h->early_fit.max_range, 0.0, rest ? 0 : h->early_fit.lds_kb);
    if (!rest) {
      DGS_HIP_TRY(h, hipEventRecord(h->ev_join, h->side_stream));
      h->side_pending = true;
    }
    return DGS_OK;
  };
  int cur = 0;
  rc = enqueue_chunk(0, h->side_build_deferred ? 2 * chunk : chunk);
  bool finished = false;
  bool first = true;
  while (rc == DGS_OK) {
    const bool more = queued < max_evals;
    if (more) rc = enqueue_chunk(cur ^ 1, chunk);
    if (rc != DGS_OK) break;
    if (first && (rc = side_build_now(h)) != DGS_OK) break;
    first = false;
    hipError_t e = hipEventSynchronize(ev[cur]);
    if (e != hipSuccess) { h->err = std::string("hipEventSynchronize: ") + hipGetErrorString(e); rc = DGS_ERR_HIP; break; }
    if (early && (rc = walk_finished(launches_upto[cur], false)) != DGS_OK) break;
    if (pairs_done(cur) >= n_pairs) { finished = true; break; }
    if (!more) break;
    cur ^= 1;
  }
  if (hd_rounds > 0) {
    hipError_t e = hipStreamWaitEvent(st, h->ev_hd_b[(hd_rounds - 1) % dgs_handle::kHdEvents], 0);
    if (e != hipSuccess && rc == DGS_OK) { h->err = std::string("hipStreamWaitEvent: ") + hipGetErrorString(e); rc = DGS_ERR_HIP; }
  }
  if (rc != DGS_OK) return rc;
  (void)finished;
  if (early) {
    if (side_join(h) != DGS_OK) return DGS_ERR_HIP;
    if ((rc = walk_finished(0, true)) != DGS_OK) return rc;
    if ((rc = nn_fitness_totals_enqueue(h, n_pairs)) != DGS_OK) return rc;
    h->early_fit.enqueued = true;
  }
  return ndt_export(h, n_pairs, results);
}

static int ndt_export(dgs_handle* h, int n_pairs, dgs_result* results) {
  hipStream_t st = h->stream;
  char* base = reinterpret_cast<char*>(h->pinned);
  const size_t off_out = ((256 + sizeof(NdtInit) * n_pairs + sizeof(void*) * n_pairs + sizeof(int) * n_pairs) + 255) & ~(size_t)255;
  NdtOut* hout = reinterpret_cast<NdtOut*>(base + off_out);
  NdtOut* dout = reinterpret_cast<NdtOut*>(h->partials.ptr);
  hipLaunchKernelGGL(ndt_export_kernel, dim3((n_pairs + 63) / 64), dim3(64), 0, st, h->pairs.ptr, n_pairs, dout);
  DGS_HIP_TRY(h, hipMemcpyAsync(hout, dout, sizeof(NdtOut) * n_pairs, hipMemcpyDeviceToHost, st));
  DGS_HIP_TRY(h, hipStreamSynchronize(st));
  DGS_HIP_TRY(h, hipGetLastError());
  int64_t evals = 0;
  for (int i = 0; i < n_pairs; i++) {
    std::memcpy(results[i].final_transformation, hout[i].T, sizeof(float) * 16);
    results[i].converged = hout[i].converged;
    results[i].iterations = hout[i].iterations;
    results[i].evaluations = hout[i].evaluations;
    results[i].status = DGS_OK;
    results[i].score = hout[i].score;
    results[i].fitness = NAN;
    evals += hout[i].evaluations;
  }
  h->last_evaluations = evals;
  return DGS_OK;
}

int ndt_trajectory(dgs_handle* h, int pair, double* out, int* len) {
  std::vector<char> buf(sizeof(NdtPair));
  DGS_HIP_TRY(h, hipStreamSynchronize(h->stream));
  DGS_HIP_TRY(h, hipMemcpy(buf.data(), h->pairs.ptr + pair, sizeof(NdtPair), hipMemcpyDeviceToHost));
  const NdtPair* st = reinterpret_cast<const NdtPair*>(buf.data());
#ifdef DGS_CLOSE_STAMPS
  const int n = kTrajCap;
#else
  const int n = std::min(st->s.traj_len, kTrajCap);
#endif
  for (int i = 0; i < n; i++)
    for (int k = 0; k < 6; k++) out[i * 6 + k] = st->traj[i][k];
  *len = n;
  return DGS_OK;
}

int ndt_probe(dgs_handle* h, const double* p6, const float* T16, double* score, double* g6, double* H36, int kind) {
  hipStream_t st = h->stream;
  NdtLaunch L{};
  const float4* src = h->src->pts.ptr;
  const int n = (int)h->ns;
  float T[16];
  if (T16) {
    std::memcpy(T, T16, sizeof(T));
  } else {
    const float rx = (float)p6[3], ry = (float)p6[4], rz = (float)p6[5];
    const float cx = (float)std::cos((double)rx), sx = (float)std::sin((double)rx), cy = (float)std::cos((double)ry), sy = (float)std::sin((double)ry),
                cz = (float)std::cos((double)rz), sz = (float)std::sin((double)rz);
    auto mul = [](float a, float b) { volatile float r = a * b; return (float)r; };
    T[0] = mul(cy, cz); T[4] = mul(-cy, sz); T[8] = sy; T[12] = (float)p6[0];
    { volatile float a = mul(cx, sz), b = mul(mul(sx, sy), cz); T[1] = a + b; }
    { volatile float a = mul(cx, cz), b = mul(mul(sx, sy), sz); T[5] = a - b; }
    T[9] = mul(-sx, cy); T[13] = (float)p6[1];
    { volatile float a = mul(sx, sz), b = mul(mul(cx, sy), cz); T[2] = a - b; }
    { volatile float a = mul(sx, cz), b = mul(mul(cx, sy), sz); T[6] = a + b; }
    T[10] = mul(cx, cy); T[14] = (float)p6[2];
    T[3] = T[7] = T[11] = 0.f; T[15] = 1.f;
  }
  int rc = ndt_setup(h, 1, &src, &n, T, p6, &L, false, kind == 0 ? 3 : kind);
  if (rc != DGS_OK) return rc;
  const NdtPlan P = plan_align(h);
  launch_derivatives(h, P, L, -1, kind == 2);
  launch_solve(h, P, L);
  char* base = reinterpret_cast<char*>(h->pinned);
  NdtPair* hp = reinterpret_cast<NdtPair*>(base + ((h->pinned_bytes - sizeof(NdtPair) - 64) & ~(size_t)63));
  DGS_HIP_TRY(h, hipMemcpyAsync(hp, h->pairs.ptr, sizeof(NdtPair), hipMemcpyDeviceToHost, st));
  DGS_HIP_TRY(h, hipStreamSynchronize(st));
  DGS_HIP_TRY(h, hipGetLastError());
  *score = hp->s.score;
  for (int k = 0; k < 6; k++) g6[k] = hp->s.grad[k];
  for (int k = 0; k < 36; k++) H36[k] = hp->s.hess[k];
  return DGS_OK;
}

}
```

delta_graph_slam_amd/csrc/ndt_voxel.hip:

```cpp
#include <hipcub/hipcub.hpp>

#include <cfloat>
#include <cmath>

#include "handle.h"
#include "small_linalg.h"

namespace dgs {

__global__ __launch_bounds__(kBlock) void minmax_kernel(const float4* __restrict__ pts, int64_t n, float* __restrict__ partial) {
  float mn[3] = {FLT_MAX, FLT_MAX, FLT_MAX}, mx[3] = {-FLT_MAX, -FLT_MAX, -FLT_MAX};
  for (int64_t i = blockIdx.x * (int64_t)blockDim.x + threadIdx.x; i < n; i += (int64_t)gridDim.x * blockDim.x) {
    const float4 p = pts[i];
    if (isfinite(p.x) && isfinite(p.y) && isfinite(p.z)) {
      mn[0] = fminf(mn[0], p.x); mn[1] = fminf(mn[1], p.y); mn[2] = fminf(mn[2], p.z);
      mx[0] = fmaxf(mx[0], p.x); mx[1] = fmaxf(mx[1], p.y); mx[2] = fmaxf(mx[2], p.z);
    }
  }
  __shared__ float sm[kBlock / kWave][6];
#pragma unroll
  for (int a = 0; a < 3; a++) {
#pragma unroll
    for (int off = 32; off > 0; off >>= 1) {
      mn[a] = fminf(mn[a], __shfl_down(mn[a], off, 64));
      mx[a] = fmaxf(mx[a], __shfl_down(mx[a], off, 64));
    }
  }
  const int lane = threadIdx.x & 63, wave = threadIdx.x >> 6;
  if (lane == 0)
    for (int a = 0; a < 3; a++) { sm[wave][a] = mn[a]; sm[wave][3 + a] = mx[a]; }
  __syncthreads();
  if (threadIdx.x < 6) {
    float v = sm[0][threadIdx.x];
    for (int w = 1; w < kBlock / kWave; w++) v = (threadIdx.x < 3) ? fminf(v, sm[w][threadIdx.x]) : fmaxf(v, sm[w][threadIdx.x]);
    partial[blockIdx.x * 6 + threadIdx.x] = v;
  }
}

__global__ void minmax_final_kernel(const float* __restrict__ partial, int nblocks, float* __restrict__ out6) {
  const int lane = threadIdx.x;
  float v[6] = {FLT_MAX, FLT_MAX, FLT_MAX, -FLT_MAX, -FLT_MAX, -FLT_MAX};
  for (int b = lane; b < nblocks; b += 64)
    for (int a = 0; a < 6; a++) v[a] = (a < 3) ? fminf(v[a], partial[b * 6 + a]) : fmaxf(v[a], partial[b * 6 + a]);
#pragma unroll
  for (int a = 0; a < 6; a++) {
#pragma unroll
    for (int off = 32; off > 0; off >>= 1) {
      const float o = __shfl_down(v[a], off, 64);
      v[a] = (a < 3) ? fminf(v[a], o) : fmaxf(v[a], o);
    }
  }
  if (lane == 0)
    for (int a = 0; a < 6; a++) out6[a] = v[a];
}

int cloud_minmax_device(dgs_handle* h, const float4* pts, int64_t n, float** d_out6, hipStream_t stream) {
  hipStream_t st = stream ? stream : h->stream;
  const int mm_blocks = (int)std::min<int64_t>((n + kBlock - 1) / kBlock, 256);
  DGS_HIP_TRY(h, h->minmax_partial.reserve((size_t)512 * 6 + 8));
  float* d_final = h->minmax_partial.ptr + (size_t)512 * 6;
  hipLaunchKernelGGL(minmax_kernel, dim3(mm_blocks), dim3(kBlock), 0, st, pts, n, h->minmax_partial.ptr);
  hipLaunchKernelGGL(minmax_final_kernel, dim3(1), dim3(64), 0, st, h->minmax_partial.ptr, mm_blocks, d_final);
  *d_out6 = d_final;
  return DGS_OK;
}

int cloud_minmax(dgs_handle* h, const float4* pts, int64_t n, float out6[6]) {
  hipStream_t st = h->stream;
  float* d_final = nullptr;
  int rc = cloud_minmax_device(h, pts, n, &d_final);
  if (rc) return rc;
  if (ensure_pinned(h, 4096) != DGS_OK) return DGS_ERR_HIP;
  float* hmm = reinterpret_cast<float*>(h->pinned);
  DGS_HIP_TRY(h, hipMemcpyAsync(hmm, d_final, 6 * sizeof(float), hipMemcpyDeviceToHost, st));
  DGS_HIP_TRY(h, hipStreamSynchronize(st));
  for (int k = 0; k < 6; k++) out6[k] = hmm[k];
  return DGS_OK;
}

__global__ __launch_bounds__(kBlock) void voxel_key_kernel(const float4* __restrict__ pts, int64_t n, VoxelGrid g,
                                                           uint32_t* __restrict__ keys, uint32_t* __restrict__ vals, int* __restrict__ clear_cells,
                                                           int64_t n_cells, int* __restrict__ clear_scalars) {
  const int64_t i = blockIdx.x * (int64_t)blockDim.x + threadIdx.x;
  if (clear_cells)
    for (int64_t c = i; c < n_cells; c += (int64_t)gridDim.x * blockDim.x) clear_cells[c] = -1;
  if (clear_scalars && i < 8) clear_scalars[i] = 0;
  if (i >= n) return;
  const float4 p = pts[i];
  uint32_t key = 0xFFFFFFFFu;
  if (isfinite(p.x) && isfinite(p.y) && isfinite(p.z)) {
    const int i0 = (int)(floorf(p.x * g.inv_leaf) - (float)g.min_b[0]);
    const int i1 = (int)(floorf(p.y * g.inv_leaf) - (float)g.min_b[1]);
    const int i2 = (int)(floorf(p.z * g.inv_leaf) - (float)g.min_b[2]);
    key = (uint32_t)(i0 + i1 * g.mul1 + i2 * g.mul2);
  }
  keys[i] = key;
  vals[i] = (uint32_t)i;
}

__global__ __launch_bounds__(kBlock) void gather_kernel(const float4* __restrict__ pts, const uint32_t* __restrict__ order, int64_t n,
                                                        float4* __restrict__ out) {
  const int64_t i = blockIdx.x * (int64_t)blockDim.x + threadIdx.x;
  if (i < n) out[i] = pts[order[i]];
}

__global__ __launch_bounds__(kBlock) void voxel_finalize_kernel(const float4* __restrict__ sorted_pts, const uint32_t* __restrict__ run_keys,
                                                                const int* __restrict__ run_counts, const int* __restrict__ run_offsets,
                                                                int* __restrict__ scalars, int min_points, double eig_mult,
                                                                int* __restrict__ cell2vox, VoxelRec* __restrict__ vox,
                                                                float4* __restrict__ centroid, double* __restrict__ dbg,
                                                                int* __restrict__ vcount, int* __restrict__ vvalid, VoxelStrictRec* __restrict__ vstrict, const int eigen_qr) {
#pragma clang fp contract(off)
  const int r = blockIdx.x * blockDim.x + threadIdx.x;
  const int num_runs = scalars[0];
  if (r >= num_runs) return;
  const uint32_t key = run_keys[r];
  const int cnt = run_counts[r];
  vcount[r] = cnt;
  vvalid[r] = 0;
  if (key == 0xFFFFFFFFu) {
    vcount[r] = 0;
    return;
  }
  const int off = run_offsets[r];
  double s[3] = {0, 0, 0}, q[6] = {0, 0, 0, 0, 0, 0};
  float cf[3] = {0, 0, 0};
  constexpr int kBatch = 24;
  for (int j0 = 0; j0 < cnt; j0 += kBatch) {
    float4 pb[kBatch];
#pragma unroll
    for (int u = 0; u < kBatch; u++) pb[u] = (j0 + u < cnt) ? sorted_pts[off + j0 + u] : make_float4(0.f, 0.f, 0.f, 0.f);
#pragma unroll
    for (int u = 0; u < kBatch; u++) {
      if (j0 + u < cnt) {
        const float4 p = pb[u];
        const double x = p.x, y = p.y, z = p.z;
        s[0] += x; s[1] += y; s[2] += z;
        q[0] += x * x; q[1] += x * y; q[2] += x * z; q[3] += y * y; q[4] += y * z; q[5] += z * z;
        cf[0] += p.x; cf[1] += p.y; cf[2] += p.z;
      }
    }
  }
  const double np = (double)cnt;
  const double mean[3] = {s[0] / np, s[1] / np, s[2] / np};
  const float fn = (float)cnt;
  double* d = dbg + (size_t)r * 12;
  d[0] = mean[0]; d[1] = mean[1]; d[2] = mean[2];
  for (int k = 0; k < 9; k++) d[3 + k] = 0.0;
  VoxelRec rec;
  rec.mean[0] = mean[0]; rec.mean[1] = mean[1]; rec.mean[2] = mean[2];
  for (int k = 0; k < 6; k++) rec.icov[k] = 0.f;
  bool valid = false;
  if (cnt >= min_points) {
    const double sq[9] = {q[0], q[1], q[2], q[1], q[3], q[4], q[2], q[4], q[5]};
    double cov[9];
    const double f = (np - 1.0) / np;
    for (int a = 0; a < 3; a++)
      for (int b = 0; b < 3; b++) cov[a * 3 + b] = ((sq[a * 3 + b] - 2.0 * (s[a] * mean[b])) / np + mean[a] * mean[b]) * f;
    double ev[3], V[9];
    if (eigen_qr) eigen_selfadjoint3_d(cov, ev, V);
    else sym_eig3_d(cov, ev, V);
    if (!(ev[0] < 0 || ev[1] < 0 || ev[2] <= 0)) {
      const double min_ev = eig_mult * ev[2];
      if (ev[0] < min_ev) {
        ev[0] = min_ev;
        if (ev[1] < min_ev) ev[1] = min_ev;
        double Vi[9], VD[9];
        inv3_d(V, Vi);
        for (int rr = 0; rr < 3; rr++)
          for (int c = 0; c < 3; c++) VD[rr * 3 + c] = V[rr * 3 + c] * ev[c];
        for (int rr = 0; rr < 3; rr++)
          for (int c = 0; c < 3; c++) cov[rr * 3 + c] = VD[rr * 3 + 0] * Vi[0 * 3 + c] + VD[rr * 3 + 1] * Vi[1 * 3 + c] + VD[rr * 3 + 2] * Vi[2 * 3 + c];
      }
      double icov[9];
      inv3_d(cov, icov);
      valid = true;
      for (int k = 0; k < 9; k++)
        if (isinf(icov[k])) valid = false;
      if (valid) {
        rec.icov[0] = (float)icov[0]; rec.icov[1] = (float)icov[1]; rec.icov[2] = (float)icov[2];
        rec.icov[3] = (float)icov[4]; rec.icov[4] = (float)icov[5]; rec.icov[5] = (float)icov[8];
        for (int k = 0; k < 9; k++) d[3 + k] = icov[k];
      }
    }
  }
  vox[r] = rec;
  {
    VoxelStrictRec sr;
    sr.mean[0] = mean[0]; sr.mean[1] = mean[1]; sr.mean[2] = mean[2];
    for (int k = 0; k < 9; k++) sr.C[k] = (float)d[3 + k];
    sr.pad = 0.f;
    vstrict[r] = sr;
  }
  centroid[r] = make_float4(cf[0] / fn, cf[1] / fn, cf[2] / fn, valid ? 1.f : 0.f);
  vvalid[r] = valid ? 1 : 0;
  cell2vox[key] = valid ? r : -1;
  if (valid) atomicAdd(&scalars[1], 1);
}

__global__ __launch_bounds__(kBlock) void voxel_centroid_kernel(const float4* __restrict__ sorted_pts, const uint32_t* __restrict__ run_keys,
                                                                const int* __restrict__ run_counts, const int* __restrict__ run_offsets,
                                                                const int* __restrict__ scalars, float4* __restrict__ out, int out_capacity) {
  const int r = blockIdx.x * blockDim.x + threadIdx.x;
  if (r >= scalars[0] || r >= out_capacity) return;
  if (run_keys[r] == 0xFFFFFFFFu) return;
  const int off = run_offsets[r], cnt = run_counts[r];
  float sx = 0.f, sy = 0.f, sz = 0.f;
  for (int j = 0; j < cnt; j++) {
    const float4 p = sorted_pts[off + j];
    sx += p.x; sy += p.y; sz += p.z;
  }
  const float fn = (float)cnt;
  out[r] = make_float4(sx / fn, sy / fn, sz / fn, 1.f);
}

__global__ void voxel_count_kernel(const uint32_t* __restrict__ run_keys, int* __restrict__ scalars) {
  const int nr = scalars[0];
  scalars[2] = (nr > 0 && run_keys[nr - 1] == 0xFFFFFFFFu) ? nr - 1 : nr;
}

int voxel_grid_filter(dgs_handle* h, const float4* in, int64_t n, float leaf, float4* out, int64_t out_capacity, int64_t* n_out) {
  hipStream_t st = h->stream;
  *n_out = 0;
  if (n == 0) return DGS_OK;
  float hmm[6];
  int rc = cloud_minmax(h, in, n, hmm);
  if (rc) return rc;
  if (!(hmm[0] <= hmm[3])) return DGS_OK;
  VoxelGrid g{};
  g.leaf = leaf;
  g.inv_leaf = 1.0f / leaf;
  int64_t cells = 1;
  for (int a = 0; a < 3; a++) {
    g.min_b[a] = (int)std::floor(hmm[a] * g.inv_leaf);
    g.max_b[a] = (int)std::floor(hmm[3 + a] * g.inv_leaf);
    g.div_b[a] = g.max_b[a] - g.min_b[a] + 1;
    cells *= (int64_t)((hmm[3 + a] - hmm[a]) * g.inv_leaf) + 1;
  }
  if (cells > INT32_MAX || (int64_t)g.div_b[0] * g.div_b[1] * g.div_b[2] > INT32_MAX) {
    h->err = "Leaf size is too small for the input dataset. Integer indices would overflow.";
    return DGS_ERR_GRID_TOO_LARGE;
  }
  g.mul1 = g.div_b[0];
  g.mul2 = g.div_b[0] * g.div_b[1];
  DGS_HIP_TRY(h, h->key_in.reserve(n));
  DGS_HIP_TRY(h, h->key_out.reserve(n));
  DGS_HIP_TRY(h, h->val_in.reserve(n));
  DGS_HIP_TRY(h, h->val_out.reserve(n));
  DGS_HIP_TRY(h, h->vg_run_keys.reserve(n));
  DGS_HIP_TRY(h, h->run_counts.reserve(n));
  DGS_HIP_TRY(h, h->run_offsets.reserve(n));
  DGS_HIP_TRY(h, h->vg_scalars.reserve(8));
  DGS_HIP_TRY(h, h->scratch_cloud.reserve(n));
  size_t t1 = 0, t2 = 0, t3 = 0;
  (void)hipcub::DeviceRadixSort::SortPairs(nullptr, t1, h->key_in.ptr, h->key_out.ptr, h->val_in.ptr, h->val_out.ptr, (int)n, 0, 32, st);
  (void)hipcub::DeviceRunLengthEncode::Encode(nullptr, t2, h->key_out.ptr, h->vg_run_keys.ptr, h->run_counts.ptr, h->vg_scalars.ptr, (int)n, st);
// ... 54 lines not shown
  head[s] = h;
}

__global__ __launch_bounds__(kBlock) void approx_runs_kernel(const int* __restrict__ head, const int* __restrict__ run_id, int n, uint32_t* __restrict__ run_start,
                                                             int* __restrict__ scalars) {
  const int s = blockIdx.x * blockDim.x + threadIdx.x;
  if (s >= n) return;
  if (head[s]) run_start[run_id[s] - 1] = (uint32_t)s;
  if (s == n - 1) scalars[0] = run_id[s];
}

__global__ __launch_bounds__(kBlock) void approx_trigger_kernel(const uint32_t* __restrict__ slots, const uint32_t* __restrict__ order,
                                                                const uint32_t* __restrict__ run_start, const int* __restrict__ scalars, int n,
                                                                uint32_t* __restrict__ trigger, uint32_t* __restrict__ run) {
  const int r = blockIdx.x * blockDim.x + threadIdx.x;
  if (r >= n) return;
  const int n_runs = scalars[0];
  uint32_t t = 0xFFFFFFFFu;
  if (r < n_runs) {
    const uint32_t s0 = run_start[r];
    const uint32_t slot = slots[s0];
    t = (uint32_t)n + slot;
    if (r + 1 < n_runs) {
      const uint32_t s1 = run_start[r + 1];
      if (slots[s1] == slot) t = order[s1];
    }
  }
  trigger[r] = t;
  run[r] = (uint32_t)r;
}

__global__ __launch_bounds__(kBlock) void approx_centroid_kernel(const float4* __restrict__ pts, const uint32_t* __restrict__ order,
                                                                 const uint32_t* __restrict__ run_start, const uint32_t* __restrict__ runs_in_output_order,
                                                                 const int* __restrict__ scalars, int n, float4* __restrict__ out, int out_capacity) {
#pragma clang fp contract(off)
  const int o = blockIdx.x * blockDim.x + threadIdx.x;
  const int n_runs = scalars[0];
  if (o >= n_runs || o >= out_capacity) return;
  const int r = (int)runs_in_output_order[o];
  const int s0 = (int)run_start[r], s1 = (r + 1 < n_runs) ? (int)run_start[r + 1] : n;
  float sx = 0.f, sy = 0.f, sz = 0.f;
  for (int s = s0; s < s1; s++) {
    const float4 p = pts[order[s]];
    sx += p.x; sy += p.y; sz += p.z;
  }
  const float fn = (float)(s1 - s0);
  out[o] = make_float4(sx / fn, sy / fn, sz / fn, 1.f);
}

int approx_voxel_grid_filter(dgs_handle* h, const float4* in, int64_t n64, float leaf, float4* out, int64_t out_capacity, int64_t* n_out) {
  hipStream_t st = h->stream;
  *n_out = 0;
  if (n64 == 0) return DGS_OK;
  const int n = (int)n64;
  const float inv_leaf = 1.0f / leaf;
  DGS_HIP_TRY(h, h->key_in.reserve(n));
  DGS_HIP_TRY(h, h->key_out.reserve(n));
  DGS_HIP_TRY(h, h->val_in.reserve(n));
  DGS_HIP_TRY(h, h->val_out.reserve(n));
  DGS_HIP_TRY(h, h->vg_run_keys.reserve(n));
  DGS_HIP_TRY(h, h->run_counts.reserve(n));
  DGS_HIP_TRY(h, h->run_offsets.reserve(n));
  DGS_HIP_TRY(h, h->vg_scalars.reserve(8));
  DGS_HIP_TRY(h, h->scratch_cloud.reserve(n));
  uint32_t* trig_sorted = reinterpret_cast<uint32_t*>(h->scratch_cloud.ptr);
  uint32_t* runs_sorted = trig_sorted + n;
  size_t t1 = 0, t2 = 0;
  (void)hipcub::DeviceRadixSort::SortPairs(nullptr, t1, h->key_in.ptr, h->key_out.ptr, h->val_in.ptr, h->val_out.ptr, n, 0, 32, st);
  (void)hipcub::DeviceScan::InclusiveSum(nullptr, t2, h->run_counts.ptr, h->run_offsets.ptr, n, st);
  DGS_HIP_TRY(h, h->cub_temp.reserve(std::max(t1, t2) + 256));
  DGS_HIP_TRY(h, hipMemsetAsync(h->vg_scalars.ptr, 0, 8 * sizeof(int), st));
  const int nb = (n + kBlock - 1) / kBlock;
  hipLaunchKernelGGL(approx_key_kernel, dim3(nb), dim3(kBlock), 0, st, in, n, inv_leaf, h->key_in.ptr, h->val_in.ptr);
  size_t tb = h->cub_temp.cap;
  DGS_HIP_TRY(h, hipcub::DeviceRadixSort::SortPairs(h->cub_temp.ptr, tb, h->key_in.ptr, h->key_out.ptr, h->val_in.ptr, h->val_out.ptr, n, 0, 9, st));
  hipLaunchKernelGGL(approx_head_kernel, dim3(nb), dim3(kBlock), 0, st, in, h->key_out.ptr, h->val_out.ptr, n, inv_leaf, h->run_counts.ptr);
  tb = h->cub_temp.cap;
  DGS_HIP_TRY(h, hipcub::DeviceScan::InclusiveSum(h->cub_temp.ptr, tb, h->run_counts.ptr, h->run_offsets.ptr, n, st));
  hipLaunchKernelGGL(approx_runs_kernel, dim3(nb), dim3(kBlock), 0, st, h->run_counts.ptr, h->run_offsets.ptr, n, h->vg_run_keys.ptr, h->vg_scalars.ptr);
  hipLaunchKernelGGL(approx_trigger_kernel, dim3(nb), dim3(kBlock), 0, st, h->key_out.ptr, h->val_out.ptr, h->vg_run_keys.ptr, h->vg_scalars.ptr, n, h->key_in.ptr,
                     h->val_in.ptr);
  tb = h->cub_temp.cap;
  DGS_HIP_TRY(h, hipcub::DeviceRadixSort::SortPairs(h->cub_temp.ptr, tb, h->key_in.ptr, trig_sorted, h->val_in.ptr, runs_sorted, n, 0, 32, st));
  hipLaunchKernelGGL(approx_centroid_kernel, dim3(nb), dim3(kBlock), 0, st, in, h->val_out.ptr, h->vg_run_keys.ptr, runs_sorted, h->vg_scalars.ptr, n, out,
                     (int)std::min<int64_t>(out_capacity, INT32_MAX));
  int* hs = reinterpret_cast<int*>(h->pinned);
  if (ensure_pinned(h, 64) != DGS_OK) return DGS_ERR_HIP;
  hs = reinterpret_cast<int*>(h->pinned);
  DGS_HIP_TRY(h, hipMemcpyAsync(hs, h->vg_scalars.ptr, 4 * sizeof(int), hipMemcpyDeviceToHost, st));
  DGS_HIP_TRY(h, hipStreamSynchronize(st));
  DGS_HIP_TRY(h, hipGetLastError());
  *n_out = hs[0];
  return DGS_OK;
}

int ndt_build_target(dgs_handle* h) {
  const int64_t n = h->nt;
  hipStream_t st = h->stream;
  const float res = (float)h->prm.ndt_resolution;
  h->grid = VoxelGrid{};
  h->grid.leaf = res;
  h->grid.inv_leaf = 1.0f / res;
  h->grid_cells = 0;
  h->counts_stale = true;
  if (n == 0) return DGS_OK;

  float hmm[6];
  int slot = prof_begin(h, DGS_K_NDT_VOXEL_BUILD);
  {
    const int rc = cloud_minmax(h, h->tgt->pts.ptr, n, hmm);
    if (rc != DGS_OK) return rc;
  }
  if (!(hmm[0] <= hmm[3])) {
    prof_end(h, DGS_K_NDT_VOXEL_BUILD, slot);
    return DGS_OK;
  }

  VoxelGrid& g = h->grid;
  int64_t cells = 1;
  for (int a = 0; a < 3; a++) {
    g.min_b[a] = (int)std::floor(hmm[a] * g.inv_leaf);
    g.max_b[a] = (int)std::floor(hmm[3 + a] * g.inv_leaf);
    g.div_b[a] = g.max_b[a] - g.min_b[a] + 1;
    const int64_t dx = (int64_t)((hmm[3 + a] - hmm[a]) * g.inv_leaf) + 1;
    cells *= dx;
  }
  const int64_t dense_cells = (int64_t)g.div_b[0] * g.div_b[1] * g.div_b[2];
  if (cells > INT32_MAX || dense_cells > INT32_MAX) {
    prof_end(h, DGS_K_NDT_VOXEL_BUILD, slot);
    h->err = "Leaf size is too small for the input dataset. Integer indices would overflow.";
    return DGS_ERR_GRID_TOO_LARGE;
  }
  g.mul1 = g.div_b[0];
  g.mul2 = g.div_b[0] * g.div_b[1];
  h->grid_cells = dense_cells;
  h->n_occupied_bound = n;

  DGS_HIP_TRY(h, h->cell2vox.reserve((size_t)dense_cells));
  DGS_HIP_TRY(h, h->key_in.reserve(n));
  DGS_HIP_TRY(h, h->key_out.reserve(n));
  DGS_HIP_TRY(h, h->val_in.reserve(n));
  DGS_HIP_TRY(h, h->val_out.reserve(n));
  DGS_HIP_TRY(h, h->run_keys.reserve(n));
  DGS_HIP_TRY(h, h->run_counts.reserve(n));
  DGS_HIP_TRY(h, h->run_offsets.reserve(n));
  DGS_HIP_TRY(h, h->dev_scalars.reserve(8));
  DGS_HIP_TRY(h, h->vox.reserve(n));
  DGS_HIP_TRY(h, h->vox_centroid.reserve(n));
  DGS_HIP_TRY(h, h->vox_dbg.reserve((size_t)n * 12));
  DGS_HIP_TRY(h, h->vox_strict.reserve(n));
  DGS_HIP_TRY(h, h->vox_count.reserve(n));
  DGS_HIP_TRY(h, h->vox_valid.reserve(n));
  DGS_HIP_TRY(h, h->scratch_cloud.reserve(n));
  size_t t1 = 0, t2 = 0, t3 = 0;
  int end_bit = 32;
  (void)hipcub::DeviceRadixSort::SortPairs(nullptr, t1, h->key_in.ptr, h->key_out.ptr, h->val_in.ptr, h->val_out.ptr, (int)n, 0, end_bit, st);
  (void)hipcub::DeviceRunLengthEncode::Encode(nullptr, t2, h->key_out.ptr, h->run_keys.ptr, h->run_counts.ptr, h->dev_scalars.ptr, (int)n, st);
  (void)hipcub::DeviceScan::ExclusiveSum(nullptr, t3, h->run_counts.ptr, h->run_offsets.ptr, (int)n, st);
  const size_t tmax = std::max(t1, std::max(t2, t3));
  DGS_HIP_TRY(h, h->cub_temp.reserve(tmax + 256));

  const int nb = (int)((n + kBlock - 1) / kBlock);
  hipLaunchKernelGGL(voxel_key_kernel, dim3(nb), dim3(kBlock), 0, st, h->tgt->pts.ptr, n, g, h->key_in.ptr, h->val_in.ptr, h->cell2vox.ptr, dense_cells,
                     h->dev_scalars.ptr);
  size_t tb = h->cub_temp.cap;
  DGS_HIP_TRY(h, hipcub::DeviceRadixSort::SortPairs(h->cub_temp.ptr, tb, h->key_in.ptr, h->key_out.ptr, h->val_in.ptr, h->val_out.ptr, (int)n, 0,
                                                    end_bit, st));
  tb = h->cub_temp.cap;
  DGS_HIP_TRY(h, hipcub::DeviceRunLengthEncode::Encode(h->cub_temp.ptr, tb, h->key_out.ptr, h->run_keys.ptr, h->run_counts.ptr,
                                                       h->dev_scalars.ptr, (int)n, st));
  tb = h->cub_temp.cap;
  DGS_HIP_TRY(h, hipcub::DeviceScan::ExclusiveSum(h->cub_temp.ptr, tb, h->run_counts.ptr, h->run_offsets.ptr, (int)n, st));
  hipLaunchKernelGGL(gather_kernel, dim3(nb), dim3(kBlock), 0, st, h->tgt->pts.ptr, h->val_out.ptr, n, h->scratch_cloud.ptr);

  hipLaunchKernelGGL(voxel_finalize_kernel, dim3(nb), dim3(kBlock), 0, st, h->scratch_cloud.ptr, h->run_keys.ptr, h->run_counts.ptr,
                     h->run_offsets.ptr, h->dev_scalars.ptr, h->prm.ndt_min_points_per_voxel, h->prm.ndt_min_covar_eigvalue_mult,
                     h->cell2vox.ptr, h->vox.ptr, h->vox_centroid.ptr, h->vox_dbg.ptr, h->vox_count.ptr, h->vox_valid.ptr, h->vox_strict.ptr,
                     h->prm.ndt_cov_eigensolver);
  prof_end(h, DGS_K_NDT_VOXEL_BUILD, slot);
  DGS_HIP_TRY(h, hipGetLastError());
  g.cell2vox = h->cell2vox.ptr;
  g.vox = h->vox.ptr;
  g.centroid = h->vox_centroid.ptr;
  return DGS_OK;
}

}
```

delta_graph_slam_amd/csrc/nn_bvh.hip:

```cpp
#include <hipcub/hipcub.hpp>

#include <cfloat>
#include <cmath>

#include <vector>
#include <cstdio>
#include "handle.h"
#include "nn_group.h"

namespace dgs {

__global__ __launch_bounds__(kBlock) void hilbert_key_kernel(const float4* __restrict__ pts, int n, const float* __restrict__ mm6,
                                                        uint32_t* __restrict__ keys, uint32_t* __restrict__ vals) {
  const int i = blockIdx.x * blockDim.x + threadIdx.x;
  if (i >= n) return;
  const float4 p = pts[i];
  float org[3] = {mm6[0], mm6[1], mm6[2]};
  float ext = fmaxf(fmaxf(mm6[3] - mm6[0], mm6[4] - mm6[1]), fmaxf(mm6[5] - mm6[2], 1e-6f));
  if (!(mm6[0] <= mm6[3])) { org[0] = org[1] = org[2] = 0.f; ext = 1.f; }
  const float scale = 1023.0f / ext;
  keys[i] = (isfinite(p.x) && isfinite(p.y) && isfinite(p.z)) ? hilbert30(p.x, p.y, p.z, org, scale) : 0x3FFFFFFFu;
  vals[i] = (uint32_t)i;
}

// ... 168 lines not shown
            if ((r & dr) == 0) {
              const int e = tid + r * kKdThreads;
              const bool up = (k == W) || ((e & k) == 0);
              const int q = r | dr;
              const bool a_gt_b = kr[r] > kr[q] || (kr[r] == kr[q] && ir[r] > ir[q]);
              if (a_gt_b == up) { const unsigned tk = kr[r]; kr[r] = kr[q]; kr[q] = tk; const uint32_t ti = ir[r]; ir[r] = ir[q]; ir[q] = ti; }
            }
          }
        } else {
          if (j >= kWave) {
            __syncthreads();
#pragma unroll
            for (int r = 0; r < kKdPer; r++) { s_key[tid + r * kKdThreads] = kr[r]; s_idx[tid + r * kKdThreads] = ir[r]; }
            __syncthreads();
          }
#pragma unroll
          for (int r = 0; r < kKdPer; r++) {
            const int e = tid + r * kKdThreads;
            unsigned pk;
            uint32_t pi;
            if (j >= kWave) { pk = s_key[e ^ j]; pi = s_idx[e ^ j]; }
            else { pk = (unsigned)__shfl_xor((int)kr[r], j); pi = (uint32_t)__shfl_xor((int)ir[r], j); }
            const bool up = (k == W) || ((e & k) == 0);
            const bool lower = (e & j) == 0;
            const bool mine_gt = kr[r] > pk || (kr[r] == pk && ir[r] > pi);
            const bool take = (lower == up) ? mine_gt : !mine_gt;
            if (take) { kr[r] = pk; ir[r] = pi; }
          }
        }
      }
    }
    __syncthreads();
#pragma unroll
    for (int r = 0; r < kKdPer; r++) { s_key[tid + r * kKdThreads] = kr[r]; s_idx[tid + r * kKdThreads] = ir[r]; }
    __syncthreads();
  }
#pragma unroll
  for (int r = 0; r < kKdPer; r++) {
    const int e = tid + r * kKdThreads;
    if (e < cnt) vals_out[base + e] = s_idx[e];
  }
}

__global__ __launch_bounds__(kBlock) void bvh_boxes_kernel(const float4* __restrict__ sorted, int n, int first, int count, int is_leaf_level,
                                                           int first_leaf, float4* __restrict__ box_lo, float4* __restrict__ box_hi) {
  const int t = blockIdx.x * blockDim.x + threadIdx.x;
  if (t >= count) return;
  const int node = first + t;
  float mn[3] = {FLT_MAX, FLT_MAX, FLT_MAX}, mx[3] = {-FLT_MAX, -FLT_MAX, -FLT_MAX};
  if (is_leaf_level) {
    const int j = node - first_leaf;
#pragma unroll
    for (int k = 0; k < kLeaf; k++) {
      const int i = j * kLeaf + k;
      if (i < n) {
        const float4 p = sorted[i];
        if (isfinite(p.x) && isfinite(p.y) && isfinite(p.z)) {
          mn[0] = fminf(mn[0], p.x); mn[1] = fminf(mn[1], p.y); mn[2] = fminf(mn[2], p.z);
          mx[0] = fmaxf(mx[0], p.x); mx[1] = fmaxf(mx[1], p.y); mx[2] = fmaxf(mx[2], p.z);
        }
      }
    }
  } else {
#pragma unroll
    for (int k = 0; k < kFan; k++) {
      const float4 l = box_lo[node * kFan + k], h = box_hi[node * kFan + k];
      mn[0] = fminf(mn[0], l.x); mn[1] = fminf(mn[1], l.y); mn[2] = fminf(mn[2], l.z);
      mx[0] = fmaxf(mx[0], h.x); mx[1] = fmaxf(mx[1], h.y); mx[2] = fmaxf(mx[2], h.z);
    }
  }
  const int parent = (node - 1) / kFan, slot = (node - 1) % kFan;
  box_lo[parent * kFan + slot] = make_float4(mn[0], mn[1], mn[2], 0.f);
  box_hi[parent * kFan + slot] = make_float4(mx[0], mx[1], mx[2], 0.f);
}


__global__ __launch_bounds__(kBlock) void nn_search_kernel(const BvhView b, const float4* __restrict__ q, int m, int* __restrict__ idx,
                                                           float* __restrict__ sq, const int rounds) {
  const int first = ((blockIdx.x * kBlock + threadIdx.x) >> 6) * (8 * rounds) + ((threadIdx.x & 63) >> 3);
  float px = 0.f, py = 0.f, pz = 0.f, prev_best = INFINITY;
  bool prev_found = false;
  for (int r = 0; r < rounds; r++) {
    const int qi = first + r * 8;
    const bool alive = qi < m;
    const float4 p = alive ? q[qi] : make_float4(0.f, 0.f, 0.f, 0.f);
    float best;
    int bi;
    nn_query_group(b, p.x, p.y, p.z, alive, nn_warm_bound_round(prev_best, prev_found, p.x, p.y, p.z, px, py, pz), best, bi);
    prev_found = alive && bi != 0x7FFFFFFF;
    prev_best = best;
    px = p.x; py = p.y; pz = p.z;
    if (alive && (threadIdx.x & 7) == 0) {
      idx[qi] = bi;
      sq[qi] = (bi != 0x7FFFFFFF) ? best : INFINITY;
    }
  }
}

struct NnPairList {
  int n;
  unsigned short id[62];
};

__global__ __launch_bounds__(kBlock) void nn_fitness_kernel(const BvhView b, const float4* const* __restrict__ src_ptrs, const int* __restrict__ sizes,
                                                            const float* __restrict__ Tbase, size_t T_stride, float max_range, float inlier_sq,
                                                            double* __restrict__ partial, int blocks_per_pair, const NnPairList list) {
  const int pair = list.n ? (int)list.id[blockIdx.y] : (int)blockIdx.y;
  const float4* __restrict__ src = src_ptrs[pair];
  const int n = sizes[pair];
  const float* T = reinterpret_cast<const float*>(reinterpret_cast<const char*>(Tbase) + (size_t)pair * T_stride);
  const float t00 = T[0], t10 = T[1], t20 = T[2], t01 = T[4], t11 = T[5], t21 = T[6], t02 = T[8], t12 = T[9], t22 = T[10], t03 = T[12],
              t13 = T[13], t23 = T[14];
  double s = 0.0, c = 0.0, inl = 0.0;
  constexpr int QPB = kBlock / 8;
  const int sub = threadIdx.x & 7;
  const int run = (n + blocks_per_pair * QPB - 1) / (blocks_per_pair * QPB);
  const int first = (blockIdx.x * (kBlock / kWave) + (threadIdx.x >> 6)) * (8 * run) + ((threadIdx.x & 63) >> 3);
  float px = 0.f, py = 0.f, pz = 0.f, prev_best = INFINITY;
  bool prev_found = false;
  for (int r = 0; r < run; r++) {
    const int i = first + r * 8;
    const bool alive = i < n;
    const float4 p = alive ? src[i] : make_float4(0.f, 0.f, 0.f, 0.f);
    const float x = affine_row_rn(t00, t01, t02, t03, p.x, p.y, p.z);
    const float y = affine_row_rn(t10, t11, t12, t13, p.x, p.y, p.z);
    const float z = affine_row_rn(t20, t21, t22, t23, p.x, p.y, p.z);
    float best;
    int bi;
    nn_query_group<false>(b, x, y, z, alive, nn_warm_bound_round(prev_best, prev_found, x, y, z, px, py, pz), best, bi);
    prev_found = alive && bi != 0x7FFFFFFF;
    prev_best = best;
    px = x; py = y; pz = z;
    if (alive && sub == 0) {
      if (bi == 0x7FFFFFFF) best = INFINITY;
      if (best <= max_range) {
        s += (double)best;
        c += 1.0;
      }
      if (best < inlier_sq) inl += 1.0;
    }
  }
  __shared__ double sm[kBlock / kWave][3];
  const int lane = threadIdx.x & 63, wave = threadIdx.x >> 6;
  s = wave_sum(s); c = wave_sum(c); inl = wave_sum(inl);
  if (lane == 0) { sm[wave][0] = s; sm[wave][1] = c; sm[wave][2] = inl; }
  __syncthreads();
  if (threadIdx.x < 3) {
    const double v = ((sm[0][threadIdx.x] + sm[1][threadIdx.x]) + sm[2][threadIdx.x]) + sm[3][threadIdx.x];
    partial[((size_t)pair * blocks_per_pair + blockIdx.x) * 4 + threadIdx.x] = v;
  }
}

__global__ __launch_bounds__(kWave) void nn_fitness_final_kernel(const double* __restrict__ partial, int blocks_per_pair, int n_pairs,
                                                                 double* __restrict__ out) {
  const int pair = blockIdx.x;
  if (pair >= n_pairs) return;
  double s = 0, c = 0, inl = 0;
  for (int b = threadIdx.x; b < blocks_per_pair; b += kWave) {
    const double* r = partial + ((size_t)pair * blocks_per_pair + b) * 4;
    s += r[0]; c += r[1]; inl += r[2];
  }
  s = wave_sum(s); c = wave_sum(c); inl = wave_sum(inl);
  if (threadIdx.x == 0) {
    out[pair * 4 + 0] = s;
    out[pair * 4 + 1] = c;
    out[pair * 4 + 2] = inl;
    out[pair * 4 + 3] = 0;
  }
}

int bvh_build(dgs_handle* h, Bvh& bvh, const float4* pts, int64_t n64, hipStream_t stream, bool kd_order) {
  hipStream_t st = stream ? stream : h->stream;
  const int n = (int)n64;
  bvh.valid = false;
  bvh.n = n;
  if (n == 0) return DGS_OK;
  h->bvh_builds++;
  const int n_leaves = (n + kLeaf - 1) / kLeaf;
  int depth = 1;
  int64_t slots = kFan;
  while (slots < n_leaves) { slots *= kFan; depth++; }
  if (depth > 8) { h->err = "cloud too large for the nearest-neighbour index (more than 8 levels)"; return DGS_ERR_UNSUPPORTED; }
  const int first_leaf = (int)((slots - 1) / (kFan - 1));
  const int n_pad = n_leaves * kLeaf;
  bvh.leaves = (int)slots;
  bvh.levels = depth;
  DGS_HIP_TRY(h, bvh.sorted.reserve(n_pad));
  DGS_HIP_TRY(h, bvh.keys.reserve(n));
  DGS_HIP_TRY(h, bvh.keys_alt.reserve(n));
  DGS_HIP_TRY(h, bvh.vals.reserve(n));
  DGS_HIP_TRY(h, bvh.vals_alt.reserve(n));
  DGS_HIP_TRY(h, bvh.node_lo.reserve((size_t)first_leaf * kFan));
  DGS_HIP_TRY(h, bvh.node_hi.reserve((size_t)first_leaf * kFan));
  const int nb = (n + kBlock - 1) / kBlock;
  const uint32_t* order = nullptr;
  if (kd_order) {
    int64_t W = 16;
    while (W < n) W <<= 1;
    const int max_seg = (int)std::max<int64_t>(1, (n + kKdChunk - 1) / kKdChunk);
    DGS_HIP_TRY(h, bvh.kd_bbox.reserve((size_t)max_seg * 6 + 6));
    size_t tb = 0;
    (void)hipcub::DeviceRadixSort::SortPairs(nullptr, tb, bvh.keys.ptr, bvh.keys_alt.ptr, bvh.vals.ptr, bvh.vals_alt.ptr, n, 0, 32, st);
    DGS_HIP_TRY(h, h->cub_temp.reserve(tb + 256));
    uint32_t* va = bvh.vals.ptr;
    uint32_t* vb = bvh.vals_alt.ptr;
    hipLaunchKernelGGL(kd_iota_kernel, dim3(nb), dim3(kBlock), 0, st, va, n, bvh.kd_bbox.ptr, 1);
    for (; W > kKdChunk; W >>= 1) {
      const int n_seg = (int)((n + W - 1) / W);
      int seg_bits = 0;
      while ((1 << seg_bits) < n_seg) seg_bits++;
      hipLaunchKernelGGL(kd_bbox_kernel, dim3(nb), dim3(kBlock), 0, st, pts, va, n, (int)W, bvh.kd_bbox.ptr);
      hipLaunchKernelGGL(kd_key_kernel, dim3(nb), dim3(kBlock), 0, st, pts, va, n, (int)W, seg_bits, bvh.kd_bbox.ptr, bvh.keys.ptr);
      size_t tbytes = h->cub_temp.cap;
      DGS_HIP_TRY(h, hipcub::DeviceRadixSort::SortPairs(h->cub_temp.ptr, tbytes, bvh.keys.ptr, bvh.keys_alt.ptr, va, vb, n, 0, 32, st));
      std::swap(va, vb);
      const int next_seg = (int)((n + W / 2 - 1) / (W / 2));
      hipLaunchKernelGGL(kd_clear_bbox_kernel, dim3((next_seg * 6 + kBlock - 1) / kBlock), dim3(kBlock), 0, st, bvh.kd_bbox.ptr, next_seg);
    }
    hipLaunchKernelGGL(kd_local_kernel, dim3(max_seg), dim3(kKdThreads), 0, st, pts, va, vb, n);
    order = vb;
  } else {
    float* d_mm = nullptr;
    int rc = cloud_minmax_device(h, pts, n, &d_mm, st);
    if (rc) return rc;
    size_t tb = 0;
    (void)hipcub::DeviceRadixSort::SortPairs(nullptr, tb, bvh.keys.ptr, bvh.keys_alt.ptr, bvh.vals.ptr, bvh.vals_alt.ptr, n, 0, 30, st);
    DGS_HIP_TRY(h, h->cub_temp.reserve(tb + 256));
    hipLaunchKernelGGL(hilbert_key_kernel, dim3(nb), dim3(kBlock), 0, st, pts, n, d_mm, bvh.keys.ptr, bvh.vals.ptr);
    tb = h->cub_temp.cap;
    DGS_HIP_TRY(h, hipcub::DeviceRadixSort::SortPairs(h->cub_temp.ptr, tb, bvh.keys.ptr, bvh.keys_alt.ptr, bvh.vals.ptr, bvh.vals_alt.ptr, n, 0, 30, st));
    order = bvh.vals_alt.ptr;
  }
  bvh.kd = kd_order;
  hipLaunchKernelGGL(gather_index_kernel, dim3((n_pad + kBlock - 1) / kBlock), dim3(kBlock), 0, st, pts, order, n, n_pad, bvh.sorted.ptr);
  hipLaunchKernelGGL(bvh_boxes_kernel, dim3((unsigned)((slots + kBlock - 1) / kBlock)), dim3(kBlock), 0, st, bvh.sorted.ptr, n, first_leaf, (int)slots, 1,
                     first_leaf, bvh.node_lo.ptr, bvh.node_hi.ptr);
  int64_t count = slots / kFan;
  for (int l = depth - 1; l >= 1; l--) {
    const int first = (int)((count - 1) / (kFan - 1));
    hipLaunchKernelGGL(bvh_boxes_kernel, dim3((unsigned)((count + kBlock - 1) / kBlock)), dim3(kBlock), 0, st, bvh.sorted.ptr, n, first, (int)count, 0,
                       first_leaf, bvh.node_lo.ptr, bvh.node_hi.ptr);
    count /= kFan;
  }
  DGS_HIP_TRY(h, hipGetLastError());
  bvh.valid = true;
  return DGS_OK;
}

BvhView make_bvh_view(const Bvh& b) {
  BvhView v;
  v.sorted = b.sorted.ptr;
  v.box_lo = b.node_lo.ptr;
  v.box_hi = b.node_hi.ptr;
  v.n = (int)b.n;
  v.depth = b.levels;
  v.first_leaf = (int)(((int64_t)b.leaves - 1) / (kFan - 1));
  return v;
}

static int ensure_target_bvh(dgs_handle* h) {
  if (side_join(h) != DGS_OK) return DGS_ERR_HIP;
  if (h->tgt->bvh.valid) return DGS_OK;
  return bvh_build(h, h->tgt->bvh, h->tgt->pts.ptr, h->nt, nullptr, (h->batch_kd || h->nn_kd_all) && !h->use_grid);
}

int ensure_target_index(dgs_handle* h, hipStream_t st) {
  int rc = DGS_OK;
  if (!h->tgt->bvh.valid) rc = bvh_build(h, h->tgt->bvh, h->tgt->pts.ptr, h->nt, st, (h->batch_kd || h->nn_kd_all) && !h->use_grid);
  if (rc == DGS_OK && h->use_grid && !h->tgt_grid.valid) rc = nn_grid_build(h, h->tgt_grid, h->tgt->bvh, h->tgt->pts.ptr, h->nt, st);
  return rc;
}

int nn_search(dgs_handle* h, const float4* queries, int64_t m, int32_t* d_idx, float* d_sq) {
  int rc = ensure_target_bvh(h);
  if (rc) return rc;
  const BvhView v = make_bvh_view(h->tgt->bvh);
  int slot = prof_begin(h, DGS_K_NN_SEARCH);
  const int rounds = (int)std::max<int64_t>(1, std::min<int64_t>(m / 65536, 8));
  const int64_t waves = (m + 8 * rounds - 1) / (8 * rounds);
  hipLaunchKernelGGL(nn_search_kernel, dim3((unsigned)((waves * kWave + kBlock - 1) / kBlock)), dim3(kBlock), 0, h->stream, v, queries, (int)m, d_idx, d_sq, rounds);
  prof_end(h, DGS_K_NN_SEARCH, slot);
  DGS_HIP_TRY(h, hipGetLastError());
  return DGS_OK;
}

int nn_fitness_batch(dgs_handle* h, int n_pairs, const float4* const* d_src_ptrs, const int* d_sizes, int max_size, const float* d_T,
                     size_t T_stride_bytes, double max_range, double inlier_sq, double* sums, int64_t* counts, int64_t* inliers) {
  h->use_grid = grid_wanted(h, (int64_t)n_pairs * max_size);
  int rc = ensure_target_bvh(h);
  if (rc == DGS_OK) rc = ensure_target_index(h);
  if (rc) return rc;
  return nn_fitness_batch_on(h, h->tgt->bvh, (h->use_grid && h->tgt_grid.valid) ? &h->tgt_grid : nullptr, n_pairs, d_src_ptrs, d_sizes, max_size, d_T, T_stride_bytes, max_range,
                             inlier_sq, sums, counts, inliers);
}

int nn_fitness_prepare(dgs_handle* h, int n_pairs, int max_size, bool grid) {
  const int full = std::max(1, (int)(((int64_t)max_size * (grid ? 1 : 8) + kBlock - 1) / kBlock));
  static const int total_blocks = std::getenv("DGS_NN_BLOCKS") ? std::atoi(std::getenv("DGS_NN_BLOCKS")) : 8192;
  const int bpp = std::max(1, std::min(full, std::max(64, total_blocks / std::max(1, n_pairs))));
  DGS_HIP_TRY(h, h->nn_partials.reserve((size_t)n_pairs * bpp * 4 + (size_t)n_pairs * 4));
  h->nn_out = h->nn_partials.ptr + (size_t)n_pairs * bpp * 4;
  h->nn_bpp = bpp;
  if (h->fit_host_cap < n_pairs) {
    if (h->fit_host) (void)hipHostFree(h->fit_host);
    h->fit_host = nullptr;
    h->fit_host_cap = 0;
    DGS_HIP_TRY(h, hipHostMalloc(reinterpret_cast<void**>(&h->fit_host), sizeof(double) * 4 * (size_t)(n_pairs + 64), hipHostMallocDefault));
    h->fit_host_cap = n_pairs + 64;
  }
  return DGS_OK;
}

void nn_fitness_enqueue(dgs_handle* h, hipStream_t st, const Bvh& index, const int* ids, int count, const float4* const* d_src_ptrs, const int* d_sizes,
                        const float* d_T, size_t T_stride_bytes, double max_range, double inlier_sq, int background_lds_kb) {
  const BvhView v = make_bvh_view(index);
  const unsigned lds = (unsigned)std::max(0, background_lds_kb) * 1024u;
  const float mr = (max_range >= (double)FLT_MAX) ? FLT_MAX : (float)max_range;
  const float iq = (inlier_sq >= (double)FLT_MAX) ? FLT_MAX : (float)inlier_sq;
  NnPairList list{};
  if (!ids) {
    hipLaunchKernelGGL(nn_fitness_kernel, dim3(h->nn_bpp, count), dim3(kBlock), 0, st, v, d_src_ptrs, d_sizes, d_T, T_stride_bytes, mr, iq, h->nn_partials.ptr,
                       h->nn_bpp, list);
    return;
  }
  constexpr int kMax = (int)(sizeof(list.id) / sizeof(list.id[0]));
  for (int o = 0; o < count; o += kMax) {
    list.n = std::min(kMax, count - o);
    for (int k = 0; k < list.n; k++) list.id[k] = (unsigned short)ids[o + k];
    hipLaunchKernelGGL(nn_fitness_kernel, dim3(h->nn_bpp, list.n), dim3(kBlock), lds, st, v, d_src_ptrs, d_sizes, d_T, T_stride_bytes, mr, iq,
                       h->nn_partials.ptr, h->nn_bpp, list);
  }
}

int nn_fitness_totals_enqueue(dgs_handle* h, int n_pairs) {
  hipStream_t st = h->stream;
  hipLaunchKernelGGL(nn_fitness_final_kernel, dim3(n_pairs), dim3(kWave), 0, st, h->nn_partials.ptr, h->nn_bpp, n_pairs, const_cast<double*>(h->nn_out));
  DGS_HIP_TRY(h, hipMemcpyAsync(h->fit_host, h->nn_out, sizeof(double) * 4 * n_pairs, hipMemcpyDeviceToHost, st));
  return DGS_OK;
}

void nn_fitness_read(const dgs_handle* h, int n_pairs, double* sums, int64_t* counts, int64_t* inliers) {
  for (int i = 0; i < n_pairs; i++) {
    sums[i] = h->fit_host[i * 4 + 0];
    counts[i] = (int64_t)h->fit_host[i * 4 + 1];
    inliers[i] = (int64_t)h->fit_host[i * 4 + 2];
  }
}

int nn_fitness_batch_on(dgs_handle* h, const Bvh& index, NnGrid* grid, int n_pairs, const float4* const* d_src_ptrs, const int* d_sizes, int max_size,
                        const float* d_T, size_t T_stride_bytes, double max_range, double inlier_sq, double* sums, int64_t* counts, int64_t* inliers) {
  hipStream_t st = h->stream;
  int rc = nn_fitness_prepare(h, n_pairs, max_size, grid != nullptr);
  if (rc) return rc;
  int slot = prof_begin(h, DGS_K_NN_SEARCH);
  if (grid) {
    const float mr = (max_range >= (double)FLT_MAX) ? FLT_MAX : (float)max_range;
    const float iq = (inlier_sq >= (double)FLT_MAX) ? FLT_MAX : (float)inlier_sq;
    const int rg = nn_grid_launch_fitness(h, *grid, index, n_pairs, d_src_ptrs, d_sizes, max_size, d_T, T_stride_bytes, mr, iq, h->nn_partials.ptr, h->nn_bpp);
    if (rg) return rg;
  } else {
    nn_fitness_enqueue(h, st, index, nullptr, n_pairs, d_src_ptrs, d_sizes, d_T, T_stride_bytes, max_range, inlier_sq, 0);
  }
  prof_end(h, DGS_K_NN_SEARCH, slot);
  rc = nn_fitness_totals_enqueue(h, n_pairs);
  if (rc) return rc;
  DGS_HIP_TRY(h, hipStreamSynchronize(st));
  DGS_HIP_TRY(h, hipGetLastError());
  nn_fitness_read(h, n_pairs, sums, counts, inliers);
  return DGS_OK;
}

int nn_fitness(dgs_handle* h, const float4* src, int64_t n, const float* T16, double max_range, double inlier_sq, double* sum, int64_t* count,
               int64_t* inliers) {
  hipStream_t st = h->stream;
  DGS_HIP_TRY(h, h->src_ptrs.reserve(1));
  DGS_HIP_TRY(h, h->src_sizes.reserve(1));
  DGS_HIP_TRY(h, h->inits.reserve(1));
  if (ensure_pinned(h, 8192) != DGS_OK) return DGS_ERR_HIP;
  char* base = reinterpret_cast<char*>(h->pinned) + 2048;
  const int ni = (int)n;
  std::memcpy(base, &src, sizeof(void*));
  std::memcpy(base + 16, &ni, sizeof(int));
  std::memcpy(base + 64, T16, sizeof(float) * 16);
  DGS_HIP_TRY(h, hipMemcpyAsync(h->src_ptrs.ptr, base, sizeof(void*), hipMemcpyHostToDevice, st));
  DGS_HIP_TRY(h, hipMemcpyAsync(h->src_sizes.ptr, base + 16, sizeof(int), hipMemcpyHostToDevice, st));
  DGS_HIP_TRY(h, hipMemcpyAsync(h->inits.ptr, base + 64, sizeof(float) * 16, hipMemcpyHostToDevice, st));
  return nn_fitness_batch(h, 1, h->src_ptrs.ptr, h->src_sizes.ptr, ni, reinterpret_cast<const float*>(h->inits.ptr), 64, max_range, inlier_sq, sum,
                          count, inliers);
}

}
```

Before: 6917 registrations/s.

## Add counting-sort voxel build, zero-copy pinned outputs, and tail fitness without early walk

Replaces the radix-sort voxel build with a dense-cell counting sort (count, tile sums, scan, scatter, rank) when the grid is small enough, which avoids the hipcub sort passes. Several small H2D/D2H copies are removed: kernels read init data directly from pinned host memory and write export, minmax and fitness results directly into pinned buffers. A memset is folded into the init kernel. Fitness is now always computed on the tail path even when early fitness is disabled. The cost is more kernel launches for the voxel build and a dense counter buffer that must be zeroed.

Measured after the change: 6949 registrations/s (median of 4 runs). No clear change (+0.5%).

```diff
diff --git a/delta_graph_slam_amd/csrc/dgs_api.hip b/delta_graph_slam_amd/csrc/dgs_api.hip
--- a/delta_graph_slam_amd/csrc/dgs_api.hip
+++ b/delta_graph_slam_amd/csrc/dgs_api.hip
@@ -428,6 +428,7 @@
   if (const char* e = std::getenv("DGS_NDT_SPECULATE")) h->ndt_speculate = std::atoi(e) != 0;
   if (const char* e = std::getenv("DGS_NDT_FIXED_SLICES")) h->ndt_fixed_slices = std::atoi(e) != 0;
   if (const char* e = std::getenv("DGS_NDT_DEAL_BY_COST")) h->ndt_deal_by_cost = std::atoi(e) != 0;
+  if (const char* e = std::getenv("DGS_NDT_VOXEL_COUNTING")) h->voxel_counting = std::atoi(e) != 0;
   if (const char* e = std::getenv("DGS_NDT_QUEUE")) h->ndt_queue_mode = std::atoi(e);
   if (const char* e = std::getenv("DGS_NDT_SCHEDULE")) h->ndt_schedule = std::atoi(e) != 0;
   if (const char* e = std::getenv("DGS_NDT_QUEUE_MIN_PAIRS")) h->ndt_queue_min_pairs = std::max(1, std::atoi(e));
@@ -494,7 +495,7 @@
   h->gitems.release(); h->vvox.release(); h->vcell2vox.release();
   h->cell2vox.release(); h->vox.release(); h->vox_centroid.release(); h->vox_dbg.release(); h->vox_strict.release(); h->vox_count.release(); h->vox_valid.release();
   h->key_in.release(); h->key_out.release(); h->val_in.release(); h->val_out.release(); h->run_keys.release();
-  h->run_counts.release(); h->run_offsets.release(); h->dev_scalars.release(); h->vg_run_keys.release(); h->vg_scalars.release(); h->minmax_partial.release(); h->cub_temp.release();
+  h->run_counts.release(); h->run_offsets.release(); h->dev_scalars.release(); h->vg_run_keys.release(); h->vg_scalars.release(); h->minmax_partial.release(); h->cub_temp.release(); h->vb_cell_cnt.release(); h->vb_tiles.release();
   h->pairs.release(); h->inits.release(); h->partials.release(); h->done_counter.release(); h->ndt_queue.release(); h->ndt_ring.release(); h->pair_blocks.release(); h->src_ptrs.release(); h->src_sizes.release();
   h->nn_partials.release(); h->scratch_cloud.release(); h->strict_rows.release(); h->strict_totals.release(); h->tgt_grid.release(); h->aux_grid.release();
   h->fc_in.release(); h->fc_out.release(); h->fc_cnt.release();
@@ -850,12 +851,13 @@
   }
   int max_n = 0;
   for (int i = 0; i < n; i++) max_n = std::max(max_n, sz[i]);
-  h->early_fit.on = h->early_fitness_enabled && compute_fitness && !h->prof.enabled && !h->use_grid && n <= 65535;
+  h->early_fit.on = compute_fitness && !h->prof.enabled && !h->use_grid && n <= 65535;
+  h->early_fit.early = h->early_fit.on && h->early_fitness_enabled;
   h->early_fit.enqueued = false;
   h->early_fit.max_range = fitness_max_range;
   h->early_fit.max_n = max_n;
   int rc = ndt_align_pairs(h, n, ptrs.data(), sz.data(), guesses16, results);
-  h->early_fit.on = false;
+  h->early_fit.on = h->early_fit.early = false;
   if (side_join(h) != DGS_OK && rc == DGS_OK) rc = DGS_ERR_HIP;
   if (rc == DGS_OK && compute_fitness && h->early_fit.enqueued) {
     std::vector<double> sums(n);
@@ -949,6 +951,7 @@
     out[2] = h->n_valid;
     out[3] = h->n_occupied;
     out[4] = h->grid_cells;
+    out[6] = h->voxel_build_counted ? 1 : 0;
   }
   out[5] = h->last_evaluations;
   return DGS_OK;
diff --git a/delta_graph_slam_amd/csrc/handle.h b/delta_graph_slam_amd/csrc/handle.h
--- a/delta_graph_slam_amd/csrc/handle.h
+++ b/delta_graph_slam_amd/csrc/handle.h
@@ -310,6 +310,10 @@
   dgs::DevBuf<int> vg_scalars;
   dgs::DevBuf<float> minmax_partial;
   dgs::DevBuf<unsigned char> cub_temp;
+  dgs::DevBuf<int> vb_cell_cnt, vb_tiles;
+  bool vb_dirty = false;
+  bool voxel_counting = true;
+  bool voxel_build_counted = false;
   int64_t grid_cells = 0;
   int64_t n_occupied = 0, n_valid = 0;
   int64_t n_occupied_bound = 0;
@@ -360,6 +364,7 @@
   int fit_host_cap = 0;
   struct EarlyFitness {
     bool on = false;
+    bool early = false;
     bool enqueued = false;
     double max_range = 0.0;
     int max_n = 0;
diff --git a/delta_graph_slam_amd/csrc/ndt_align.hip b/delta_graph_slam_amd/csrc/ndt_align.hip
--- a/delta_graph_slam_amd/csrc/ndt_align.hip
+++ b/delta_graph_slam_amd/csrc/ndt_align.hip
@@ -35,8 +35,9 @@
 __global__ void ndt_init_kernel(NdtPair* __restrict__ pairs, const NdtInit* __restrict__ inits, int n_pairs, const NdtConsts c, int probe,
                                 int* __restrict__ done_counter, const float4* const* __restrict__ stage_ptrs, const int* __restrict__ stage_sizes,
                                 const float4** __restrict__ src_ptrs, int* __restrict__ src_sizes, int* __restrict__ queue, const int queue_slices0,
-                                char* __restrict__ ring, const int ring_rounds) {
+                                char* __restrict__ ring, const int ring_rounds, int* __restrict__ clear_pair_blocks) {
   const int i = blockIdx.x * blockDim.x + threadIdx.x;
+  if (clear_pair_blocks && i < n_pairs) clear_pair_blocks[i] = 0;
   if (i < 16) done_counter[i] = 0;
   if (queue && i == 0) *queue_ctl(queue) = (unsigned long long)n_pairs;
   if (queue && i < kQueueStatInts) queue[2 * (n_pairs + 2) + i] = 0;
@@ -468,7 +469,6 @@
   if (h->consts.strict_order) DGS_HIP_TRY(h, h->strict_totals.reserve((size_t)n_pairs * kStrictPad));
   if (h->consts.strict_order == DGS_NDT_ORDER_UPSTREAM_SEQUENTIAL) DGS_HIP_TRY(h, h->strict_rows.reserve((size_t)n_pairs * strict_rows_pair_stride(h, L)));
   DGS_HIP_TRY(h, h->pair_blocks.reserve(n_pairs));
-  if (h->consts.strict_order == DGS_NDT_ORDER_UPSTREAM) DGS_HIP_TRY(h, hipMemsetAsync(h->pair_blocks.ptr, 0, sizeof(int) * n_pairs, st));
   DGS_HIP_TRY(h, h->done_counter.reserve(16));
   const size_t off_init = 256;
   const size_t off_ptr = off_init + sizeof(NdtInit) * n_pairs;
@@ -502,15 +502,12 @@
   }
   std::memcpy(base + off_ptr, src_ptrs_host, sizeof(void*) * n_pairs);
   std::memcpy(base + off_size, sizes_host, sizeof(int) * n_pairs);
-  const size_t stage_bytes = off_size + sizeof(int) * n_pairs - off_init;
-  DGS_HIP_TRY(h, h->inits.reserve((stage_bytes + sizeof(NdtInit) - 1) / sizeof(NdtInit)));
-  DGS_HIP_TRY(h, hipMemcpyAsync(h->inits.ptr, hin, stage_bytes, hipMemcpyHostToDevice, st));
-  const char* dstage = reinterpret_cast<const char*>(h->inits.ptr);
-  hipLaunchKernelGGL(ndt_init_kernel, dim3((n_pairs + 63) / 64), dim3(64), 0, st, h->pairs.ptr, h->inits.ptr, n_pairs, h->consts, probe_p6 ? probe_kind : 0,
-                     h->done_counter.ptr, reinterpret_cast<const float4* const*>(dstage + (off_ptr - off_init)),
-                     reinterpret_cast<const int*>(dstage + (off_size - off_init)), h->src_ptrs.ptr, h->src_sizes.ptr,
+  hipLaunchKernelGGL(ndt_init_kernel, dim3((n_pairs + 63) / 64), dim3(64), 0, st, h->pairs.ptr, hin, n_pairs, h->consts, probe_p6 ? probe_kind : 0,
+                     h->done_counter.ptr, reinterpret_cast<const float4* const*>(base + off_ptr), reinterpret_cast<const int*>(base + off_size),
+                     h->src_ptrs.ptr, h->src_sizes.ptr,
                      L.queue_workers > 0 ? h->ndt_queue.ptr : nullptr, L.queue_workers > 0 ? ndt_queue_slices(0, L.queue_base, L.cap_blocks) : 0,
-                     reinterpret_cast<char*>(h->ndt_ring.ptr), h->ndt_ring_rounds);
+                     reinterpret_cast<char*>(h->ndt_ring.ptr), h->ndt_ring_rounds,
+                     h->consts.strict_order == DGS_NDT_ORDER_UPSTREAM ? h->pair_blocks.ptr : nullptr);
   if (is_pcl_ndt(h)) pcl_ndt_init_tables(h, n_pairs, st);
   return DGS_OK;
 }
@@ -640,7 +637,8 @@
     for (int i = 0; i < n_pairs; i++) n += reinterpret_cast<volatile int*>(h->done_flags)[i] != 0;
     return n;
   };
-  const bool early = h->early_fit.on && fused_flags;
+  const bool tail_fit = h->early_fit.on && fused_flags;
+  const bool early = tail_fit && h->early_fit.early;
   std::vector<char> walked(early ? n_pairs : 0, 0);
   const float* fit_T = reinterpret_cast<const float*>(reinterpret_cast<const char*>(h->pairs.ptr) + offsetof(NdtPair, final_T));
   std::vector<int> ready;
@@ -684,9 +682,14 @@
   }
   if (rc != DGS_OK) return rc;
   (void)finished;
-  if (early) {
+  if (tail_fit) {
     if (side_join(h) != DGS_OK) return DGS_ERR_HIP;
-    if ((rc = walk_finished(0, true)) != DGS_OK) return rc;
+    if (!h->tgt->bvh.valid) { h->err = "fitness walk: the target's index was not built"; return DGS_ERR_HIP; }
+    if (early) {
+      if ((rc = walk_finished(0, true)) != DGS_OK) return rc;
+    } else {
+      nn_fitness_enqueue(h, st, h->tgt->bvh, nullptr, n_pairs, h->src_ptrs.ptr, h->src_sizes.ptr, fit_T, sizeof(NdtPair), h->early_fit.max_range, 0.0, 0);
+    }
     if ((rc = nn_fitness_totals_enqueue(h, n_pairs)) != DGS_OK) return rc;
     h->early_fit.enqueued = true;
   }
@@ -698,9 +701,7 @@
   char* base = reinterpret_cast<char*>(h->pinned);
   const size_t off_out = ((256 + sizeof(NdtInit) * n_pairs + sizeof(void*) * n_pairs + sizeof(int) * n_pairs) + 255) & ~(size_t)255;
   NdtOut* hout = reinterpret_cast<NdtOut*>(base + off_out);
-  NdtOut* dout = reinterpret_cast<NdtOut*>(h->partials.ptr);
-  hipLaunchKernelGGL(ndt_export_kernel, dim3((n_pairs + 63) / 64), dim3(64), 0, st, h->pairs.ptr, n_pairs, dout);
-  DGS_HIP_TRY(h, hipMemcpyAsync(hout, dout, sizeof(NdtOut) * n_pairs, hipMemcpyDeviceToHost, st));
+  hipLaunchKernelGGL(ndt_export_kernel, dim3((n_pairs + 63) / 64), dim3(64), 0, st, h->pairs.ptr, n_pairs, hout);
   DGS_HIP_TRY(h, hipStreamSynchronize(st));
   DGS_HIP_TRY(h, hipGetLastError());
   int64_t evals = 0;
diff --git a/delta_graph_slam_amd/csrc/ndt_voxel.hip b/delta_graph_slam_amd/csrc/ndt_voxel.hip
--- a/delta_graph_slam_amd/csrc/ndt_voxel.hip
+++ b/delta_graph_slam_amd/csrc/ndt_voxel.hip
@@ -4,6 +4,7 @@
 #include <cmath>
 
 #include "handle.h"
+#include "ndt_voxel_plan.h"
 #include "small_linalg.h"
 
 namespace dgs {
@@ -67,12 +68,12 @@
 
 int cloud_minmax(dgs_handle* h, const float4* pts, int64_t n, float out6[6]) {
   hipStream_t st = h->stream;
-  float* d_final = nullptr;
-  int rc = cloud_minmax_device(h, pts, n, &d_final);
-  if (rc) return rc;
   if (ensure_pinned(h, 4096) != DGS_OK) return DGS_ERR_HIP;
   float* hmm = reinterpret_cast<float*>(h->pinned);
-  DGS_HIP_TRY(h, hipMemcpyAsync(hmm, d_final, 6 * sizeof(float), hipMemcpyDeviceToHost, st));
+  const int mm_blocks = (int)std::min<int64_t>((n + kBlock - 1) / kBlock, 256);
+  DGS_HIP_TRY(h, h->minmax_partial.reserve((size_t)512 * 6 + 8));
+  hipLaunchKernelGGL(minmax_kernel, dim3(mm_blocks), dim3(kBlock), 0, st, pts, n, h->minmax_partial.ptr);
+  hipLaunchKernelGGL(minmax_final_kernel, dim3(1), dim3(64), 0, st, h->minmax_partial.ptr, mm_blocks, hmm);
   DGS_HIP_TRY(h, hipStreamSynchronize(st));
   for (int k = 0; k < 6; k++) out6[k] = hmm[k];
   return DGS_OK;
@@ -102,6 +103,158 @@
                                                         float4* __restrict__ out) {
   const int64_t i = blockIdx.x * (int64_t)blockDim.x + threadIdx.x;
   if (i < n) out[i] = pts[order[i]];
+}
+
+__device__ __forceinline__ uint32_t voxel_key_of(const float4 p, const VoxelGrid& g) {
+  if (!(isfinite(p.x) && isfinite(p.y) && isfinite(p.z))) return 0xFFFFFFFFu;
+  const int i0 = (int)(floorf(p.x * g.inv_leaf) - (float)g.min_b[0]);
+  const int i1 = (int)(floorf(p.y * g.inv_leaf) - (float)g.min_b[1]);
+  const int i2 = (int)(floorf(p.z * g.inv_leaf) - (float)g.min_b[2]);
+  return (uint32_t)(i0 + i1 * g.mul1 + i2 * g.mul2);
+}
+
+__global__ __launch_bounds__(kBlock) void voxel_cell_count_kernel(const float4* __restrict__ pts, int64_t n, VoxelGrid g, uint32_t n_cells,
+                                                                  uint32_t* __restrict__ keys, uint32_t* __restrict__ slots, int* __restrict__ cell_cnt) {
+  const int64_t i = blockIdx.x * (int64_t)blockDim.x + threadIdx.x;
+  const int lane = threadIdx.x & (kWave - 1);
+  const bool active = i < n;
+  uint32_t key = 0xFFFFFFFFu;
+  if (active) {
+    key = voxel_key_of(pts[i], g);
+    if (key >= n_cells) key = 0xFFFFFFFFu;
+  }
+  const uint32_t c = (key == 0xFFFFFFFFu) ? n_cells : key;
+  unsigned long long todo = __ballot(active);
+  int leader = lane, rank = 0, group = 1;
+  while (todo) {
+    const int l = __ffsll((long long)todo) - 1;
+    const uint32_t cl = (uint32_t)__shfl((int)c, l, kWave);
+    const bool mine = active && c == cl;
+    const unsigned long long m = __ballot(mine);
+    if (mine) {
+      leader = l;
+      rank = __popcll(m & ((1ull << lane) - 1ull));
+      group = __popcll(m);
+    }
+    todo &= ~m;
+  }
+  int base = 0;
+  if (active && leader == lane) base = atomicAdd(&cell_cnt[c], group);
+  base = __shfl(base, leader, kWave);
+  if (active) {
+    keys[i] = key;
+    slots[i] = (uint32_t)(base + rank);
+  }
+}
+
+__global__ __launch_bounds__(kBlock) void voxel_tile_sum_kernel(const int* __restrict__ cell_cnt, int* __restrict__ tile_pts, int* __restrict__ tile_occ) {
+  constexpr int kPer = kVbTile / kBlock;
+  static_assert(kPer == 8, "two 16-byte loads per lane");
+  __shared__ int sm_pts[kBlock / kWave], sm_occ[kBlock / kWave];
+  const int t = threadIdx.x, lane = t & (kWave - 1), wave = t / kWave;
+  const int4* cp = reinterpret_cast<const int4*>(cell_cnt + (size_t)blockIdx.x * kVbTile + (size_t)t * kPer);
+  const int4 a = cp[0], b = cp[1];
+  int pts = a.x + a.y + a.z + a.w + b.x + b.y + b.z + b.w;
+  int occ = (a.x != 0) + (a.y != 0) + (a.z != 0) + (a.w != 0) + (b.x != 0) + (b.y != 0) + (b.z != 0) + (b.w != 0);
+#pragma unroll
+  for (int off = 32; off > 0; off >>= 1) { pts += __shfl_xor(pts, off, kWave); occ += __shfl_xor(occ, off, kWave); }
+  if (lane == 0) { sm_pts[wave] = pts; sm_occ[wave] = occ; }
+  __syncthreads();
+  if (t == 0) {
+    pts = 0; occ = 0;
+#pragma unroll
+    for (int w = 0; w < kBlock / kWave; w++) { pts += sm_pts[w]; occ += sm_occ[w]; }
+    tile_pts[blockIdx.x] = pts;
+    tile_occ[blockIdx.x] = occ;
+  }
+}
+
+__global__ __launch_bounds__(kBlock) void voxel_cell_scan_kernel(int* __restrict__ cell_cnt, const int* __restrict__ tile_pts, const int* __restrict__ tile_occ,
+                                                                 uint32_t n_cells, uint32_t* __restrict__ run_keys, int* __restrict__ run_counts,
+                                                                 int* __restrict__ run_offsets, int* __restrict__ cell2vox, int* __restrict__ scalars) {
+  constexpr int kPer = kVbTile / kBlock;
+  static_assert(kPer == 8, "two 16-byte loads per lane");
+  __shared__ int sm_pts[kBlock / kWave], sm_occ[kBlock / kWave];
+  const int t = threadIdx.x, lane = t & (kWave - 1), wave = t / kWave;
+  const int tile = blockIdx.x;
+  int base_pts = 0, base_occ = 0;
+  for (int b = t; b < tile; b += kBlock) { base_pts += tile_pts[b]; base_occ += tile_occ[b]; }
+#pragma unroll
+  for (int off = 32; off > 0; off >>= 1) { base_pts += __shfl_xor(base_pts, off, kWave); base_occ += __shfl_xor(base_occ, off, kWave); }
+  if (lane == 0) { sm_pts[wave] = base_pts; sm_occ[wave] = base_occ; }
+  __syncthreads();
+  base_pts = 0; base_occ = 0;
+#pragma unroll
+  for (int w = 0; w < kBlock / kWave; w++) { base_pts += sm_pts[w]; base_occ += sm_occ[w]; }
+  __syncthreads();
+  const size_t first = (size_t)tile * kVbTile + (size_t)t * kPer;
+  int4* cp = reinterpret_cast<int4*>(cell_cnt + first);
+  const int4 a = cp[0], b = cp[1];
+  const int c[kPer] = {a.x, a.y, a.z, a.w, b.x, b.y, b.z, b.w};
+  cp[0] = make_int4(0, 0, 0, 0);
+  cp[1] = make_int4(0, 0, 0, 0);
+  int my_pts = 0, my_occ = 0;
+#pragma unroll
+  for (int k = 0; k < kPer; k++) { my_pts += c[k]; my_occ += c[k] != 0; }
+  int inc_pts = my_pts, inc_occ = my_occ;
+#pragma unroll
+  for (int off = 1; off < kWave; off <<= 1) {
+    const int p = __shfl_up(inc_pts, off, kWave), o = __shfl_up(inc_occ, off, kWave);
+    if (lane >= off) { inc_pts += p; inc_occ += o; }
+  }
+  if (lane == kWave - 1) { sm_pts[wave] = inc_pts; sm_occ[wave] = inc_occ; }
+  __syncthreads();
+  int off_pts = base_pts + inc_pts - my_pts, run = base_occ + inc_occ - my_occ;
+  for (int w = 0; w < wave; w++) { off_pts += sm_pts[w]; run += sm_occ[w]; }
+#pragma unroll
+  for (int k = 0; k < kPer; k++) {
+    const size_t cell = first + k;
+    if (c[k] != 0) {
+      run_keys[run] = (cell == n_cells) ? 0xFFFFFFFFu : (uint32_t)cell;
+      run_counts[run] = c[k];
+      run_offsets[run] = off_pts;
+    }
+    if (cell < n_cells) cell2vox[cell] = (c[k] != 0) ? run : -1;
+    else if (cell == n_cells) scalars[3] = (c[k] != 0) ? run : -1;
+    if (c[k] != 0) { run++; off_pts += c[k]; }
+  }
+  if (tile == (int)gridDim.x - 1 && t == kBlock - 1) {
+    scalars[0] = run;
+    scalars[1] = 0;
+    scalars[2] = off_pts;
+    for (int k = 4; k < 8; k++) scalars[k] = 0;
+  }
+}
+
+__global__ __launch_bounds__(kBlock) void voxel_cell_scatter_kernel(const uint32_t* __restrict__ keys, const uint32_t* __restrict__ slots, int64_t n,
+                                                                    const int* __restrict__ cell2vox, const int* __restrict__ run_offsets,
+                                                                    uint32_t* __restrict__ list) {
+  const int64_t i = blockIdx.x * (int64_t)blockDim.x + threadIdx.x;
+  if (i >= n) return;
+  const uint32_t key = keys[i];
+  if (key == 0xFFFFFFFFu) return;
+  list[(size_t)run_offsets[cell2vox[key]] + slots[i]] = (uint32_t)i;
+}
+
+__global__ __launch_bounds__(kBlock) void voxel_cell_rank_kernel(const float4* __restrict__ pts, const uint32_t* __restrict__ keys,
+                                                                 const uint32_t* __restrict__ list, int64_t n, const int* __restrict__ cell2vox,
+                                                                 const int* __restrict__ run_counts, const int* __restrict__ run_offsets,
+                                                                 const int* __restrict__ scalars, float4* __restrict__ sorted_pts) {
+  const int64_t p = blockIdx.x * (int64_t)blockDim.x + threadIdx.x;
+  const int nf_run = scalars[3];
+  const int64_t n_listed = (nf_run >= 0) ? (int64_t)run_offsets[nf_run] : n;
+  if (p >= n_listed) return;
+  const uint32_t idx = list[p];
+  const int r = cell2vox[keys[idx]];
+  const int off = run_offsets[r], cnt = run_counts[r];
+  const uint32_t* l = list + off;
+  int rank = 0, j = 0;
+  for (; j + 4 <= cnt; j += 4) {
+    const uint32_t a = l[j], b = l[j + 1], c = l[j + 2], d = l[j + 3];
+    rank += (a < idx) + (b < idx) + (c < idx) + (d < idx);
+  }
+  for (; j < cnt; j++) rank += l[j] < idx;
+  sorted_pts[(size_t)off + rank] = pts[idx];
 }
 
 __global__ __launch_bounds__(kBlock) void voxel_finalize_kernel(const float4* __restrict__ sorted_pts, const uint32_t* __restrict__ run_keys,
@@ -462,6 +615,45 @@
   DGS_HIP_TRY(h, h->vox_count.reserve(n));
   DGS_HIP_TRY(h, h->vox_valid.reserve(n));
   DGS_HIP_TRY(h, h->scratch_cloud.reserve(n));
+  const int nb = (int)((n + kBlock - 1) / kBlock);
+  auto finalize = [&]() {
+    hipLaunchKernelGGL(voxel_finalize_kernel, dim3(nb), dim3(kBlock), 0, st, h->scratch_cloud.ptr, h->run_keys.ptr, h->run_counts.ptr,
+                       h->run_offsets.ptr, h->dev_scalars.ptr, h->prm.ndt_min_points_per_voxel, h->prm.ndt_min_covar_eigvalue_mult,
+                       h->cell2vox.ptr, h->vox.ptr, h->vox_centroid.ptr, h->vox_dbg.ptr, h->vox_count.ptr, h->vox_valid.ptr, h->vox_strict.ptr,
+                       h->prm.ndt_cov_eigensolver);
+    prof_end(h, DGS_K_NDT_VOXEL_BUILD, slot);
+    g.cell2vox = h->cell2vox.ptr;
+    g.vox = h->vox.ptr;
+    g.centroid = h->vox_centroid.ptr;
+  };
+
+  const VoxelBuildPlan vb = plan_voxel_build(dense_cells, n, h->voxel_counting);
+  h->voxel_build_counted = vb.counting;
+  if (vb.counting) {
+    const bool grown = h->vb_cell_cnt.cap < vb.counter_ints;
+    DGS_HIP_TRY(h, h->vb_cell_cnt.reserve(vb.counter_ints));
+    DGS_HIP_TRY(h, h->vb_tiles.reserve(vb.tile_ints));
+    if (grown || h->vb_dirty) DGS_HIP_TRY(h, hipMemsetAsync(h->vb_cell_cnt.ptr, 0, h->vb_cell_cnt.cap * sizeof(int), st));
+    h->vb_dirty = true;
+    int* tile_pts = h->vb_tiles.ptr;
+    int* tile_occ = h->vb_tiles.ptr + vb.tiles;
+    const uint32_t n_cells = (uint32_t)dense_cells;
+    hipLaunchKernelGGL(voxel_cell_count_kernel, dim3(nb), dim3(kBlock), 0, st, h->tgt->pts.ptr, n, g, n_cells, h->key_in.ptr, h->val_in.ptr,
+                       h->vb_cell_cnt.ptr);
+    hipLaunchKernelGGL(voxel_tile_sum_kernel, dim3(vb.tiles), dim3(kBlock), 0, st, h->vb_cell_cnt.ptr, tile_pts, tile_occ);
+    hipLaunchKernelGGL(voxel_cell_scan_kernel, dim3(vb.tiles), dim3(kBlock), 0, st, h->vb_cell_cnt.ptr, tile_pts, tile_occ, n_cells, h->run_keys.ptr,
+                       h->run_counts.ptr, h->run_offsets.ptr, h->cell2vox.ptr, h->dev_scalars.ptr);
+    hipLaunchKernelGGL(voxel_cell_scatter_kernel, dim3(nb), dim3(kBlock), 0, st, h->key_in.ptr, h->val_in.ptr, n, h->cell2vox.ptr, h->run_offsets.ptr,
+                       h->val_out.ptr);
+    hipLaunchKernelGGL(voxel_cell_rank_kernel, dim3(nb), dim3(kBlock), 0, st, h->tgt->pts.ptr, h->key_in.ptr, h->val_out.ptr, n, h->cell2vox.ptr,
+                       h->run_counts.ptr, h->run_offsets.ptr, h->dev_scalars.ptr, h->scratch_cloud.ptr);
+    DGS_HIP_TRY(h, hipGetLastError());
+    h->vb_dirty = false;
+    finalize();
+    DGS_HIP_TRY(h, hipGetLastError());
+    return DGS_OK;
+  }
+
   size_t t1 = 0, t2 = 0, t3 = 0;
   int end_bit = 32;
   (void)hipcub::DeviceRadixSort::SortPairs(nullptr, t1, h->key_in.ptr, h->key_out.ptr, h->val_in.ptr, h->val_out.ptr, (int)n, 0, end_bit, st);
@@ -470,7 +662,6 @@
   const size_t tmax = std::max(t1, std::max(t2, t3));
   DGS_HIP_TRY(h, h->cub_temp.reserve(tmax + 256));
 
-  const int nb = (int)((n + kBlock - 1) / kBlock);
   hipLaunchKernelGGL(voxel_key_kernel, dim3(nb), dim3(kBlock), 0, st, h->tgt->pts.ptr, n, g, h->key_in.ptr, h->val_in.ptr, h->cell2vox.ptr, dense_cells,
                      h->dev_scalars.ptr);
   size_t tb = h->cub_temp.cap;
@@ -483,15 +674,8 @@
   DGS_HIP_TRY(h, hipcub::DeviceScan::ExclusiveSum(h->cub_temp.ptr, tb, h->run_counts.ptr, h->run_offsets.ptr, (int)n, st));
   hipLaunchKernelGGL(gather_kernel, dim3(nb), dim3(kBlock), 0, st, h->tgt->pts.ptr, h->val_out.ptr, n, h->scratch_cloud.ptr);
 
-  hipLaunchKernelGGL(voxel_finalize_kernel, dim3(nb), dim3(kBlock), 0, st, h->scratch_cloud.ptr, h->run_keys.ptr, h->run_counts.ptr,
-                     h->run_offsets.ptr, h->dev_scalars.ptr, h->prm.ndt_min_points_per_voxel, h->prm.ndt_min_covar_eigvalue_mult,
-                     h->cell2vox.ptr, h->vox.ptr, h->vox_centroid.ptr, h->vox_dbg.ptr, h->vox_count.ptr, h->vox_valid.ptr, h->vox_strict.ptr,
-                     h->prm.ndt_cov_eigensolver);
-  prof_end(h, DGS_K_NDT_VOXEL_BUILD, slot);
+  finalize();
   DGS_HIP_TRY(h, hipGetLastError());
-  g.cell2vox = h->cell2vox.ptr;
-  g.vox = h->vox.ptr;
-  g.centroid = h->vox_centroid.ptr;
   return DGS_OK;
 }
 
diff --git a/delta_graph_slam_amd/csrc/ndt_voxel_plan.h b/delta_graph_slam_amd/csrc/ndt_voxel_plan.h
--- /dev/null
+++ b/delta_graph_slam_amd/csrc/ndt_voxel_plan.h
@@ -0,0 +1,42 @@
+#pragma once
+#include <algorithm>
+#include <cstddef>
+#include <cstdint>
+
+namespace dgs {
+
+constexpr int kVbTile = 2048;
+constexpr int64_t kVbFloorCells = (int64_t)1 << 22;
+constexpr int64_t kVbCellsPerPoint = 64;
+constexpr int64_t kVbMaxCells = (int64_t)1 << 24;
+
+struct VoxelBuildPlan {
+  bool counting = false;
+  int64_t entries = 0;
+  int tiles = 0;
+  size_t counter_ints = 0;
+  size_t tile_ints = 0;
+};
+
+inline bool voxel_build_counts(int64_t dense_cells, int64_t n, bool enabled) {
+  if (!enabled || dense_cells < 1 || n < 1) return false;
+  if (dense_cells > kVbMaxCells) return false;
+  const int64_t by_points = (n > kVbMaxCells / kVbCellsPerPoint) ? kVbMaxCells : n * kVbCellsPerPoint;
+  return dense_cells <= std::max(kVbFloorCells, by_points);
+}
+
+inline VoxelBuildPlan plan_voxel_build(int64_t dense_cells, int64_t n, bool enabled) {
+  VoxelBuildPlan P;
+  P.counting = voxel_build_counts(dense_cells, n, enabled);
+  if (!P.counting) return P;
+  P.entries = dense_cells + 1;
+  P.tiles = (int)((P.entries + kVbTile - 1) / kVbTile);
+  P.counter_ints = (size_t)P.tiles * kVbTile;
+  P.tile_ints = (size_t)P.tiles * 2;
+  return P;
+}
+
+inline int64_t voxel_tile_first(int t) { return (int64_t)t * kVbTile; }
+inline int voxel_tile_of(int64_t cell) { return (int)(cell / kVbTile); }
+
+}
diff --git a/delta_graph_slam_amd/csrc/nn_bvh.hip b/delta_graph_slam_amd/csrc/nn_bvh.hip
--- a/delta_graph_slam_amd/csrc/nn_bvh.hip
+++ b/delta_graph_slam_amd/csrc/nn_bvh.hip
@@ -344,7 +344,7 @@
 }
 
 __global__ __launch_bounds__(kWave) void nn_fitness_final_kernel(const double* __restrict__ partial, int blocks_per_pair, int n_pairs,
-                                                                 double* __restrict__ out) {
+                                                                 double* __restrict__ out, double* __restrict__ host_out) {
   const int pair = blockIdx.x;
   if (pair >= n_pairs) return;
   double s = 0, c = 0, inl = 0;
@@ -358,6 +358,10 @@
     out[pair * 4 + 1] = c;
     out[pair * 4 + 2] = inl;
     out[pair * 4 + 3] = 0;
+    host_out[pair * 4 + 0] = s;
+    host_out[pair * 4 + 1] = c;
+    host_out[pair * 4 + 2] = inl;
+    host_out[pair * 4 + 3] = 0;
   }
 }
 
@@ -526,8 +530,9 @@
 
 int nn_fitness_totals_enqueue(dgs_handle* h, int n_pairs) {
   hipStream_t st = h->stream;
-  hipLaunchKernelGGL(nn_fitness_final_kernel, dim3(n_pairs), dim3(kWave), 0, st, h->nn_partials.ptr, h->nn_bpp, n_pairs, const_cast<double*>(h->nn_out));
-  DGS_HIP_TRY(h, hipMemcpyAsync(h->fit_host, h->nn_out, sizeof(double) * 4 * n_pairs, hipMemcpyDeviceToHost, st));
+  hipLaunchKernelGGL(nn_fitness_final_kernel, dim3(n_pairs), dim3(kWave), 0, st, h->nn_partials.ptr, h->nn_bpp, n_pairs, const_cast<double*>(h->nn_out),
+                     h->fit_host);
+  DGS_HIP_TRY(h, hipGetLastError());
   return DGS_OK;
 }
 
```
